# marl/l3embedding

Hardware: AMD Instinct MI355X
Metric: AVC training pairs/sec (1s audio + 224x224 frame) (higher is better)
Workload: dtype f32; 1 GPU; full cnn_L3_melspec2 AVC training step (audio+vision+fusion, fwd+bwd+Adam), batch 64 per GPU, global batch 64, fp32, inputs resident in HBM; global_batch=64, parallelism=dp1, fp32_conv=f4x4

## Files before the change

### include/l3hip.h

```cpp
#ifndef L3HIP_H
#define L3HIP_H

#include <stdint.h>

#ifdef __cplusplus
extern "C" {
#endif

#define L3_OK 0
#define L3_EINVAL (-1)
#define L3_EHIP (-2)
#define L3_ENOMEM (-3)
#define L3_ESTATE (-4)
#define L3_ECOMM (-5)

#define L3_MODEL_CNN_L3_ORIG 0
#define L3_MODEL_TINY_L3 1
#define L3_MODEL_CNN_L3_KAPREDBINPUTBN 2
#define L3_MODEL_CNN_L3_MELSPEC1 3
#define L3_MODEL_CNN_L3_MELSPEC2 4

typedef struct l3_engine l3_engine;

#define L3_DTYPE_F32 0
// ... 84 lines not shown
#define L3_COMM_ID_BYTES 128
int l3_comm_unique_id(void *id128);
int l3_comm_init(l3_engine *e, const void *id128, int world, int rank);
int l3_comm_destroy(l3_engine *e);
int l3_comm_info(const l3_engine *e, int *world, int *rank, char *library_path, int path_cap);
int l3_comm_version(void);
int l3_comm_allreduce_host(l3_engine *e, double *vals, int n, int op);
int l3_step_dp(l3_engine *e, float lr);
int l3_comm_timing(l3_engine *e, int on);
int l3_comm_timing_read(l3_engine *e, double *exposed_ms, double *span_ms, double *bucket_ms, int cap, int *steps);

int l3_grad_arena_dev(l3_engine *e, void **dev_ptr, int64_t *numel);
int l3_bucket_range(const l3_engine *e, int bucket, int64_t *offset, int64_t *numel);
int l3_bn_stats_pack_dev(l3_engine *e, void **send_dev, int64_t *numel);
int l3_bn_stats_replicas_dev(l3_engine *e, int world, void **gathered_dev);

int l3_embed_audio(l3_engine *e, const float *audio, int64_t n, int pool_h, int pool_w, float *out);
int l3_embed_vision(l3_engine *e, const float *video, int64_t n, int pool_h, int pool_w, float *out);
int64_t l3_embed_dim(const l3_engine *e, int vision, int pool_h, int pool_w);
int l3_embed_audio_frames(l3_engine *e, const float *samples, int64_t n_samples, const int64_t *table,
                          int64_t n_frames, int pool_h, int pool_w, float *out);
int l3_embed_audio_clips_resampled(l3_engine *e, const float *native, int64_t n_native, const int64_t *clips,
                                   int64_t n_clips, const double *half_window, int64_t n_window, int num_table,
                                   int64_t n_samples, const int64_t *table, int64_t n_frames, int pool_h, int pool_w,
                                   float *out);
int l3_embed_vision_frames(l3_engine *e, const uint8_t *pixels, int64_t n_bytes, const int64_t *table, int64_t n_frames,
                           int pool_h, int pool_w, float *out);

int l3_get_activation(l3_engine *e, const char *name, float *dst, int64_t numel);
int l3_activation_numel(l3_engine *e, const char *name, int64_t *numel);
int l3_sync(l3_engine *e);
int l3_profile_enable(l3_engine *e, int on);
int l3_set_tower_overlap(l3_engine *e, int on);
int l3_profile_read(l3_engine *e, int family, double *ms, int64_t *launches, double *flops);
int l3_profile_read_executed(l3_engine *e, int family, double *flops);
int l3_profile_read_bytes(l3_engine *e, int family, double *bytes);

#define L3_OP_BF16_STORED 2
#define L3_OP_BF16_STORED_OUT 3
int l3_op_conv2d_fwd_dt(int device, int dtype, const float *x, const float *w, const float *b, float *y,
                        int n, int h, int wd, int cin, int cout, int kh, int kw, int same);
int l3_op_conv2d_bwd_dt(int device, int dtype, const float *x, const float *w, const float *dy, float *dx,
                        float *dw, float *db, int n, int h, int wd, int cin, int cout, int kh, int kw, int same);
int l3_op_conv2d_fwd(int device, const float *x, const float *w, const float *b, float *y,
                     int n, int h, int wd, int cin, int cout, int kh, int kw, int same);
int l3_op_conv2d_bwd(int device, const float *x, const float *w, const float *dy,
                     float *dx, float *dw, float *db,
                     int n, int h, int wd, int cin, int cout, int kh, int kw, int same);
int l3_op_bn_relu_fwd(int device, const float *x, const float *gamma, const float *beta,
                      float *y, float *mean, float *var, int64_t rows, int c, int relu, int x_bf16);
int l3_op_bn_relu_bwd(int device, const float *x, const float *y, const float *dy,
                      const float *gamma, const float *beta, const float *mean, const float *var,
                      float *dx, float *dgamma, float *dbeta, int64_t rows, int c, int relu, int x_bf16);
int l3_op_bn_relu_pool2_fwd(int device, const float *x, const float *gamma, const float *beta, float *p,
                            float *mean, float *var, int n, int h, int wd, int c, int same, int relu_mode, int x_bf16);
int l3_op_bn_relu_pool2_bwd(int device, const float *x, const float *gamma, const float *beta, const float *dp,
                            float *dx, float *dgamma, float *dbeta, float *dbias, int n, int h, int wd, int c,
                            int same, int relu_mode, int x_bf16);
int l3_op_maxpool_fwd(int device, const float *x, float *y, int n, int h, int wd, int c,
                      int ph, int pw, int sh, int sw, int same);
int l3_op_maxpool_bwd(int device, const float *x, const float *dy, float *dx, int n, int h,
                      int wd, int c, int ph, int pw, int sh, int sw, int same);
int l3_op_frontend(int device, int model_type, const float *audio, int n, int db_max_scope, float *out);
int l3_op_gather_frames(int device, const float *samples, int64_t n_samples, const int64_t *table,
                        int64_t n_frames, float *frames);
int l3_op_image_frames(int device, const uint8_t *pixels, int64_t n_bytes, const int64_t *table, int64_t n_frames,
                       uint8_t *out_u8, float *out_f32);
int l3_op_resample(int device, const float *x, int64_t n_in, int64_t sr_orig, int64_t sr_new, const double *half_window,
                   int64_t n_window, int num_table, int64_t t0, int64_t n_out, float *y);
int l3_op_resample_clips(int device, const float *x, int64_t n_in, const int64_t *clips, int64_t n_clips, int64_t sr_new,
                         const double *half_window, int64_t n_window, int num_table, int64_t n_samples, int copy_equal,
                         float *y);
int l3_op_bn_stats_from_partials(int device, const float *part, int nblk, int c, const float *pivot, int64_t rows,
                                 float eps, float *mean, float *var);
int l3_op_conv2d_fwd_stats(int device, int dtype, const float *x, const float *w, const float *b, float *y, float *part, int *nblk,
                           float *mean, float *var, int n, int h, int wd, int cin, int cout, int kh, int kw, int same,
                           int stat_mode);
int l3_op_conv2d_dgrad_bn_bwd(int device, int dtype, const float *dy, const float *w, const float *bn_x, const float *gamma,
                              const float *beta, const float *mean, const float *var, float *dx, float *part, int *nblk,
                              float *dgamma, float *dbeta, int n, int h, int wd, int cin, int cout, int kh, int kw, int same,
                              int relu, int64_t bn_rows);
int l3_op_bn_relu_pool2_fwd_xwin(int device, const float *x, const float *gamma, const float *beta, float *p, float *mean,
                                 float *var, float *xwin, int n, int h, int wd, int c, int same, int relu_mode, int x_bf16);
int l3_op_preprocess(int device, const uint8_t *video_u8, int64_t nv, float *video,
                     const int16_t *audio_i16, int64_t na, float *audio);
int l3_op_augment_video(int device, const uint8_t *u8, int n, int h, int w, const l3_augment_params *params,
                        uint8_t *out_u8, float *out_f32);
int l3_op_augment_audio(int device, const int16_t *i16, int n, int t, const double *u, int16_t *out_i16, float *out_f32,
                        double *gains);

typedef struct l3_mlp l3_mlp;
int l3_mlp_create(int device, int D, int C, int batch, float weight_decay, uint64_t seed, l3_mlp **m);
void l3_mlp_destroy(l3_mlp *m);
int64_t l3_mlp_param_count(const l3_mlp *m);
int l3_mlp_set_data(l3_mlp *m, const float *X_train, const int32_t *y_train, int64_t n_train,
                    const float *X_valid, const int32_t *y_valid, int64_t n_valid);
int l3_mlp_epoch(l3_mlp *m, const int32_t *perm, float lr, int64_t t0, double *stats_out);
int l3_mlp_predict(l3_mlp *m, const float *X, int64_t n, float *probs_out);
int l3_mlp_get_weights(l3_mlp *m, float *dst, int64_t n);
int l3_mlp_set_weights(l3_mlp *m, const float *src, int64_t n);

int l3_op_mlp_dense_fwd(int device, const float *x, int64_t n_x, const int32_t *idx, int rows, int K, int N, const float *w,
                        const float *b, int relu, float *y);
int l3_op_mlp_dense_bwd_x(int device, const float *dy, const float *w, const float *h, int rows, int K, int N, float *dx);
int l3_op_mlp_wgrad(int device, const float *x, int64_t n_x, const int32_t *idx, int rows, int K, int N, const float *dy, float *dw,
                    float *db);
int l3_op_mlp_wgrad_adam(int device, const float *x, int64_t n_x, const int32_t *idx, int rows, int K, int N, const float *dy,
                         float *w, float *b, float *mw, float *vw, float *mb, float *vb, float weight_decay, float lr_t,
                         float *w2_out);
int l3_op_mlp_softmax_ce(int device, const float *z, const int32_t *labels, int rows, int C, float gscale, float *probs, float *dz,
                         float *ce, float *correct);
int l3_op_adam(int device, float *p, const float *g, float *m, float *v, int64_t n, int64_t n_l2, float l2x2, float lr_t);
int l3_op_adam_scaled(int device, float *p, const float *g, float *m, float *v, int64_t n, int64_t n_l2, float l2x2, float lr_t,
                      float b1, float b2, float eps, float gscale);
int l3_op_arena_fold(int device, float *acc, float *g, int64_t total, int64_t off, int64_t n, int mode);

int l3_op_head_dense_fwd(int device, const float *x, const float *w, const float *b, float *y, int B, int K, int N, int relu);
int l3_op_head_dense_bwd(int device, const float *x, const float *w, const float *dy, float *dw, float *db, float *dx, int B,
                         int K, int N);
int l3_op_softmax_ce2(int device, const float *logits, const float *labels, int B, float gscale, float *probs, float *dlogits,
                      float *stats);
int l3_op_sumsq(int device, const float *base, int64_t n_base, const int64_t *off, const int64_t *n, int count, int multi,
                float *out);
int l3_op_bn_moving_update(int device, int entries, const int32_t *c, const int64_t *slot_off, int64_t n_slots, float *moving,
                           float *biased, const float *batch, const float *gathered, int64_t n_gathered, int replicas,
                           int64_t stride, float momentum, int zero_debias, int64_t step, float *packed, int64_t n_packed);

#define L3_SVM_LINEAR 0
#define L3_SVM_POLY 1
#define L3_SVM_RBF 2
#define L3_SVM_SIGMOID 3
#define L3_SVM_DEFAULT_WS 64
#define L3_SVM_LOCAL_REL 0.1
typedef struct l3_svm_kernel {
    int32_t kind, degree;
    double gamma, coef0;
} l3_svm_kernel;
typedef struct l3_svm l3_svm;
int l3_svm_create(int device, l3_svm **m);
void l3_svm_destroy(l3_svm *m);
int l3_svm_set_data(l3_svm *m, const float *X, int64_t n, int D);
int l3_svm_fit(l3_svm *m, const l3_svm_kernel *k, double C, double tol, int64_t max_iter, int n_prob, const int64_t *prob_off,
               const int32_t *rows, const int8_t *signs, int q, double *alpha_out, double *rho_out, int64_t *updates_out,
               int32_t *outer_out, double *gap_out);
int l3_svm_fit_costs(l3_svm *m, const l3_svm_kernel *k, const double *C, double tol, int64_t max_iter, int n_prob,
                     const int64_t *prob_off, const int32_t *rows, const int8_t *signs, int q, double *alpha_out, double *rho_out,
                     int64_t *updates_out, int32_t *outer_out, double *gap_out);
int l3_svm_cv_decision(l3_svm *m, const l3_svm_kernel *k, int n_jobs, const int64_t *held_off, const int32_t *held_rows,
                       const int64_t *sv_off, const int64_t *sv_neg, const int32_t *sv_rows, const double *coef, const double *rho,
                       double *dec_out);
int l3_svm_decision(l3_svm *m, const l3_svm_kernel *k, const float *X, const int32_t *x_idx, int64_t n, int D, const float *SV,
                    const int32_t *sv_idx, int64_t n_sv, int n_class, const int64_t *sv_start, const double *coef,
                    const double *rho, double *dec_out);
int l3_op_svm_kernel_rows(int device, const l3_svm_kernel *k, const float *x, int64_t n_x, int D, const int32_t *a_idx, int na,
                          const int32_t *b_idx, int nb, float *out);
int l3_op_svm_smo(int device, const float *K, const int8_t *y, int q, double C, double eps, double local_rel, int64_t max_updates,
                  double *alpha, const double *grad, int64_t *updates_out);
int l3_svm_set_data_dev(l3_svm *m, const struct l3_feat *f, int64_t lo, int64_t hi);
int l3_svm_get_rows(l3_svm *m, const int32_t *idx, int64_t n, float *out);
int l3_svm_set_model(l3_svm *m, const l3_svm_kernel *k, const float *SV, const int32_t *sv_idx, int64_t n_sv, int D, int n_class,
                     const int64_t *sv_start, const double *coef, const double *rho, const double *probA, const double *probB);
int l3_svm_score(l3_svm *m, const float *X, const int32_t *x_idx, const struct l3_feat *feat, int64_t lo, int64_t hi, int64_t n,
                 int D, const int32_t *labels, const int64_t *files, int64_t n_files, int32_t *pred_out, double *ovr_out,
                 double *hinge_sum_out, double *proba_out, double *file_proba_out, int32_t *file_pred_out);
int l3_op_svm_tail(int device, const double *dec, int64_t n, int n_class, const double *probA, const double *probB,
                   const int32_t *labels, const int64_t *files, int64_t n_files, int32_t *pred_out, double *ovr_out,
// ... 127 lines not shown
```

### l3embedding_amd/_lib.py

```python
import ctypes as C
import os

import numpy as np

from . import _build

MODEL_IDS = {
    'cnn_L3_orig': 0,
    'tiny_L3': 1,
    'cnn_L3_kapredbinputbn': 2,
    'cnn_L3_melspec1': 3,
    'cnn_L3_melspec2': 4,
}

FAMILIES = ('conv_fwd', 'conv_dgrad', 'conv_wgrad', 'elementwise', 'frontend', 'head', 'adam')


DTYPES = {'f32': 0, 'fp32': 0, 'float32': 0, 'bf16': 1}
FP32_CONV = {'f4x4': 0, 'f2x2': 1, 'f2x2_bf16x6': 2}
DP_MOVING = {'replicas': 0, 'rank_local': 1}
OP_DTYPES = dict(DTYPES, bf16_stored=2, bf16_stored_out=3)


class L3Config(C.Structure):
# ... 46 lines not shown
                               C.POINTER(C.c_float), C.POINTER(C.c_float)]),
    'l3_upload_batch': (C.c_int, [C.c_void_p, C.c_void_p, C.c_void_p, C.c_void_p]),
    'l3_upload_batch_raw': (C.c_int, [C.c_void_p, C.c_void_p, C.c_void_p, C.c_void_p]),
    'l3_tower_step': (C.c_int, [C.c_void_p, C.c_int, C.c_int]),
    'l3_stage_batch_raw': (C.c_int, [C.c_void_p, C.c_void_p, C.c_void_p, C.c_void_p]),
    'l3_upload_batch_raw_aug': (C.c_int, [C.c_void_p, C.c_void_p, C.c_void_p, C.c_void_p, C.c_void_p, C.c_void_p]),
    'l3_stage_batch_raw_aug': (C.c_int, [C.c_void_p, C.c_void_p, C.c_void_p, C.c_void_p, C.c_void_p, C.c_void_p]),
    'l3_batch_gains': (C.c_int, [C.c_void_p, C.c_void_p]),
    'l3_step_forward': (C.c_int, [C.c_void_p, C.c_int]),
    'l3_step_bucket_count': (C.c_int, [C.c_void_p]),
    'l3_step_backward_bucket': (C.c_int, [C.c_void_p, C.c_int]),
    'l3_step_update': (C.c_int, [C.c_void_p, C.c_float, C.c_float]),
    'l3_step_resident': (C.c_int, [C.c_void_p, C.c_float]),
    'l3_replicas_upload': (C.c_int, [C.c_void_p, C.c_void_p, C.c_void_p, C.c_void_p, C.c_int]),
    'l3_replicas_upload_raw': (C.c_int, [C.c_void_p, C.c_void_p, C.c_void_p, C.c_void_p, C.c_int]),
    'l3_replicas_stage_raw': (C.c_int, [C.c_void_p, C.c_void_p, C.c_void_p, C.c_void_p, C.c_int]),
    'l3_replicas_upload_raw_aug': (C.c_int, [C.c_void_p] * 6 + [C.c_int]),
    'l3_replicas_stage_raw_aug': (C.c_int, [C.c_void_p] * 6 + [C.c_int]),
    'l3_step_replicas': (C.c_int, [C.c_void_p, C.c_float]),
    'l3_eval_replicas': (C.c_int, [C.c_void_p, C.POINTER(C.c_float), C.POINTER(C.c_float)]),
    'l3_step_results': (C.c_int, [C.c_void_p, C.POINTER(C.c_float), C.POINTER(C.c_float), C.c_void_p, C.c_void_p]),
    'l3_step_results_enqueue': (C.c_int, [C.c_void_p, C.c_int, C.c_int]),
    'l3_step_results_wait': (C.c_int, [C.c_void_p, C.c_int, C.POINTER(C.c_float), C.POINTER(C.c_float)]),
    'l3_comm_unique_id': (C.c_int, [C.c_void_p]),
    'l3_comm_init': (C.c_int, [C.c_void_p, C.c_void_p, C.c_int, C.c_int]),
    'l3_comm_destroy': (C.c_int, [C.c_void_p]),
    'l3_comm_info': (C.c_int, [C.c_void_p, C.POINTER(C.c_int), C.POINTER(C.c_int), C.c_char_p, C.c_int]),
    'l3_comm_allreduce_host': (C.c_int, [C.c_void_p, C.POINTER(C.c_double), C.c_int, C.c_int]),
    'l3_step_dp': (C.c_int, [C.c_void_p, C.c_float]),
    'l3_comm_timing': (C.c_int, [C.c_void_p, C.c_int]),
    'l3_comm_timing_read': (C.c_int, [C.c_void_p, C.POINTER(C.c_double), C.POINTER(C.c_double), C.POINTER(C.c_double), C.c_int, C.POINTER(C.c_int)]),
    'l3_grad_arena_dev': (C.c_int, [C.c_void_p, C.POINTER(C.c_void_p), C.POINTER(C.c_int64)]),
    'l3_bucket_range': (C.c_int, [C.c_void_p, C.c_int, C.POINTER(C.c_int64), C.POINTER(C.c_int64)]),
    'l3_embed_audio': (C.c_int, [C.c_void_p, C.c_void_p, C.c_int64, C.c_int, C.c_int, C.c_void_p]),
    'l3_embed_vision': (C.c_int, [C.c_void_p, C.c_void_p, C.c_int64, C.c_int, C.c_int, C.c_void_p]),
    'l3_embed_dim': (C.c_int64, [C.c_void_p, C.c_int, C.c_int, C.c_int]),
    'l3_embed_audio_frames': (C.c_int, [C.c_void_p, C.c_void_p, C.c_int64, C.c_void_p, C.c_int64, C.c_int, C.c_int,
                                        C.c_void_p]),
    'l3_embed_audio_clips_resampled': (C.c_int, [C.c_void_p, C.c_void_p, C.c_int64, C.c_void_p, C.c_int64, C.c_void_p,
                                                 C.c_int64, C.c_int, C.c_int64, C.c_void_p, C.c_int64, C.c_int, C.c_int,
                                                 C.c_void_p]),
    'l3_embed_audio_frames_dev': (C.c_int, [C.c_void_p, C.c_void_p, C.c_int64, C.c_void_p, C.c_int64, C.c_int, C.c_int,
                                            C.c_void_p, C.c_int64]),
    'l3_embed_audio_clips_resampled_dev': (C.c_int, [C.c_void_p, C.c_void_p, C.c_int64, C.c_void_p, C.c_int64, C.c_void_p,
                                                     C.c_int64, C.c_int, C.c_int64, C.c_void_p, C.c_int64, C.c_int, C.c_int,
                                                     C.c_void_p, C.c_int64]),
    'l3_embed_vision_frames': (C.c_int, [C.c_void_p, C.c_void_p, C.c_int64, C.c_void_p, C.c_int64, C.c_int, C.c_int,
                                         C.c_void_p]),
    'l3_embed_vision_frames_dev': (C.c_int, [C.c_void_p, C.c_void_p, C.c_int64, C.c_void_p, C.c_int64, C.c_int, C.c_int,
                                             C.c_void_p, C.c_int64]),
    'l3_get_activation': (C.c_int, [C.c_void_p, C.c_char_p, C.c_void_p, C.c_int64]),
    'l3_activation_numel': (C.c_int, [C.c_void_p, C.c_char_p, C.POINTER(C.c_int64)]),
    'l3_sync': (C.c_int, [C.c_void_p]),
    'l3_profile_enable': (C.c_int, [C.c_void_p, C.c_int]),
    'l3_set_tower_overlap': (C.c_int, [C.c_void_p, C.c_int]),
    'l3_profile_read_executed': (C.c_int, [C.c_void_p, C.c_int, C.POINTER(C.c_double)]),
    'l3_profile_read_bytes': (C.c_int, [C.c_void_p, C.c_int, C.POINTER(C.c_double)]),
    'l3_profile_read': (C.c_int, [C.c_void_p, C.c_int, C.POINTER(C.c_double), C.POINTER(C.c_int64),
                                  C.POINTER(C.c_double)]),
    'l3_op_conv2d_fwd': (C.c_int, [C.c_int, C.c_void_p, C.c_void_p, C.c_void_p, C.c_void_p] + [C.c_int] * 8),
    'l3_op_conv2d_fwd_dt': (C.c_int, [C.c_int, C.c_int, C.c_void_p, C.c_void_p, C.c_void_p, C.c_void_p] + [C.c_int] * 8),
    'l3_op_conv2d_bwd_dt': (C.c_int, [C.c_int, C.c_int] + [C.c_void_p] * 6 + [C.c_int] * 8),
    'l3_op_conv2d_bwd': (C.c_int, [C.c_int] + [C.c_void_p] * 6 + [C.c_int] * 8),
    'l3_op_bn_relu_fwd': (C.c_int, [C.c_int] + [C.c_void_p] * 6 + [C.c_int64, C.c_int, C.c_int, C.c_int]),
    'l3_op_bn_relu_bwd': (C.c_int, [C.c_int] + [C.c_void_p] * 10 + [C.c_int64, C.c_int, C.c_int, C.c_int]),
    'l3_op_bn_relu_pool2_fwd': (C.c_int, [C.c_int] + [C.c_void_p] * 6 + [C.c_int] * 7),
    'l3_op_bn_relu_pool2_bwd': (C.c_int, [C.c_int] + [C.c_void_p] * 8 + [C.c_int] * 7),
    'l3_op_maxpool_fwd': (C.c_int, [C.c_int, C.c_void_p, C.c_void_p] + [C.c_int] * 9),
    'l3_op_maxpool_bwd': (C.c_int, [C.c_int, C.c_void_p, C.c_void_p, C.c_void_p] + [C.c_int] * 9),
    'l3_op_frontend': (C.c_int, [C.c_int, C.c_int, C.c_void_p, C.c_int, C.c_int, C.c_void_p]),
    'l3_op_gather_frames': (C.c_int, [C.c_int, C.c_void_p, C.c_int64, C.c_void_p, C.c_int64, C.c_void_p]),
    'l3_op_image_frames': (C.c_int, [C.c_int, C.c_void_p, C.c_int64, C.c_void_p, C.c_int64, C.c_void_p, C.c_void_p]),
    'l3_op_resample': (C.c_int, [C.c_int, C.c_void_p, C.c_int64, C.c_int64, C.c_int64, C.c_void_p, C.c_int64, C.c_int,
                                 C.c_int64, C.c_int64, C.c_void_p]),
    'l3_op_resample_clips': (C.c_int, [C.c_int, C.c_void_p, C.c_int64, C.c_void_p, C.c_int64, C.c_int64, C.c_void_p, C.c_int64,
                                       C.c_int, C.c_int64, C.c_int, C.c_void_p]),
    'l3_op_bn_stats_from_partials': (C.c_int, [C.c_int, C.c_void_p, C.c_int, C.c_int, C.c_void_p, C.c_int64, C.c_float,
                                               C.c_void_p, C.c_void_p]),
    'l3_op_conv2d_fwd_stats': (C.c_int, [C.c_int, C.c_int] + [C.c_void_p] * 5 + [C.POINTER(C.c_int), C.c_void_p, C.c_void_p] +
                               [C.c_int] * 9),
    'l3_op_conv2d_dgrad_bn_bwd': (C.c_int, [C.c_int, C.c_int] + [C.c_void_p] * 9 + [C.POINTER(C.c_int), C.c_void_p, C.c_void_p] +
                                  [C.c_int] * 9 + [C.c_int64]),
    'l3_op_bn_relu_pool2_fwd_xwin': (C.c_int, [C.c_int] + [C.c_void_p] * 7 + [C.c_int] * 7),
    'l3_op_preprocess': (C.c_int, [C.c_int, C.c_void_p, C.c_int64, C.c_void_p, C.c_void_p, C.c_int64, C.c_void_p]),
    'l3_op_augment_video': (C.c_int, [C.c_int, C.c_void_p, C.c_int, C.c_int, C.c_int, C.c_void_p, C.c_void_p, C.c_void_p]),
    'l3_op_augment_audio': (C.c_int, [C.c_int, C.c_void_p, C.c_int, C.c_int, C.c_void_p, C.c_void_p, C.c_void_p, C.c_void_p]),
    'l3_mlp_create': (C.c_int, [C.c_int, C.c_int, C.c_int, C.c_int, C.c_float, C.c_uint64, C.POINTER(C.c_void_p)]),
    'l3_mlp_destroy': (None, [C.c_void_p]),
    'l3_mlp_param_count': (C.c_int64, [C.c_void_p]),
    'l3_mlp_set_data': (C.c_int, [C.c_void_p, C.c_void_p, C.c_void_p, C.c_int64, C.c_void_p, C.c_void_p, C.c_int64]),
    'l3_mlp_epoch': (C.c_int, [C.c_void_p, C.c_void_p, C.c_float, C.c_int64, C.POINTER(C.c_double)]),
    'l3_mlp_predict': (C.c_int, [C.c_void_p, C.c_void_p, C.c_int64, C.c_void_p]),
    'l3_mlp_get_weights': (C.c_int, [C.c_void_p, C.c_void_p, C.c_int64]),
    'l3_mlp_set_weights': (C.c_int, [C.c_void_p, C.c_void_p, C.c_int64]),
    'l3_op_mlp_dense_fwd': (C.c_int, [C.c_int, C.c_void_p, C.c_int64, C.c_void_p, C.c_int, C.c_int, C.c_int, C.c_void_p,
                                      C.c_void_p, C.c_int, C.c_void_p]),
    'l3_op_mlp_dense_bwd_x': (C.c_int, [C.c_int, C.c_void_p, C.c_void_p, C.c_void_p, C.c_int, C.c_int, C.c_int, C.c_void_p]),
    'l3_op_mlp_wgrad': (C.c_int, [C.c_int, C.c_void_p, C.c_int64, C.c_void_p, C.c_int, C.c_int, C.c_int, C.c_void_p,
                                  C.c_void_p, C.c_void_p]),
    'l3_op_mlp_wgrad_adam': (C.c_int, [C.c_int, C.c_void_p, C.c_int64, C.c_void_p, C.c_int, C.c_int, C.c_int, C.c_void_p]
                             + [C.c_void_p] * 6 + [C.c_float, C.c_float, C.c_void_p]),
    'l3_op_mlp_softmax_ce': (C.c_int, [C.c_int, C.c_void_p, C.c_void_p, C.c_int, C.c_int, C.c_float] + [C.c_void_p] * 4),
    'l3_op_adam': (C.c_int, [C.c_int] + [C.c_void_p] * 4 + [C.c_int64, C.c_int64, C.c_float, C.c_float]),
    'l3_op_adam_scaled': (C.c_int, [C.c_int] + [C.c_void_p] * 4 + [C.c_int64, C.c_int64] + [C.c_float] * 6),
    'l3_op_arena_fold': (C.c_int, [C.c_int, C.c_void_p, C.c_void_p, C.c_int64, C.c_int64, C.c_int64, C.c_int]),
    'l3_op_head_dense_fwd': (C.c_int, [C.c_int] + [C.c_void_p] * 4 + [C.c_int] * 4),
    'l3_op_head_dense_bwd': (C.c_int, [C.c_int] + [C.c_void_p] * 6 + [C.c_int] * 3),
    'l3_op_softmax_ce2': (C.c_int, [C.c_int, C.c_void_p, C.c_void_p, C.c_int, C.c_float] + [C.c_void_p] * 3),
    'l3_op_sumsq': (C.c_int, [C.c_int, C.c_void_p, C.c_int64, C.c_void_p, C.c_void_p, C.c_int, C.c_int, C.c_void_p]),
    'l3_op_bn_moving_update': (C.c_int, [C.c_int, C.c_int, C.c_void_p, C.c_void_p, C.c_int64] + [C.c_void_p] * 4
                               + [C.c_int64, C.c_int, C.c_int64, C.c_float, C.c_int, C.c_int64, C.c_void_p, C.c_int64]),
    'l3_svm_create': (C.c_int, [C.c_int, C.POINTER(C.c_void_p)]),
    'l3_svm_destroy': (None, [C.c_void_p]),
    'l3_svm_set_data': (C.c_int, [C.c_void_p, C.c_void_p, C.c_int64, C.c_int]),
    'l3_svm_fit': (C.c_int, [C.c_void_p, C.c_void_p, C.c_double, C.c_double, C.c_int64, C.c_int] + [C.c_void_p] * 3
                   + [C.c_int] + [C.c_void_p] * 5),
    'l3_svm_fit_costs': (C.c_int, [C.c_void_p, C.c_void_p, C.c_void_p, C.c_double, C.c_int64, C.c_int] + [C.c_void_p] * 3
                         + [C.c_int] + [C.c_void_p] * 5),
    'l3_svm_cv_decision': (C.c_int, [C.c_void_p, C.c_void_p, C.c_int] + [C.c_void_p] * 8),
    'l3_op_svm_sigmoid_train': (C.c_int, [C.c_int, C.c_int] + [C.c_void_p] * 6),
    'l3_svm_decision': (C.c_int, [C.c_void_p, C.c_void_p, C.c_void_p, C.c_void_p, C.c_int64, C.c_int, C.c_void_p, C.c_void_p,
                                  C.c_int64, C.c_int] + [C.c_void_p] * 4),
    'l3_op_svm_kernel_rows': (C.c_int, [C.c_int, C.c_void_p, C.c_void_p, C.c_int64, C.c_int, C.c_void_p, C.c_int, C.c_void_p,
                                        C.c_int, C.c_void_p]),
    'l3_op_svm_smo': (C.c_int, [C.c_int, C.c_void_p, C.c_void_p, C.c_int, C.c_double, C.c_double, C.c_double, C.c_int64,
                                C.c_void_p, C.c_void_p, C.c_void_p]),
    'l3_svm_set_data_dev': (C.c_int, [C.c_void_p, C.c_void_p, C.c_int64, C.c_int64]),
    'l3_svm_get_rows': (C.c_int, [C.c_void_p, C.c_void_p, C.c_int64, C.c_void_p]),
    'l3_svm_set_model': (C.c_int, [C.c_void_p, C.c_void_p, C.c_void_p, C.c_void_p, C.c_int64, C.c_int, C.c_int] + [C.c_void_p] * 5),
    'l3_svm_score': (C.c_int, [C.c_void_p, C.c_void_p, C.c_void_p, C.c_void_p, C.c_int64, C.c_int64, C.c_int64, C.c_int, C.c_void_p,
                               C.c_void_p, C.c_int64] + [C.c_void_p] * 6),
    'l3_op_svm_tail': (C.c_int, [C.c_int, C.c_void_p, C.c_int64, C.c_int, C.c_void_p, C.c_void_p, C.c_void_p, C.c_void_p, C.c_int64]
                       + [C.c_void_p] * 8),
    'l3_vggish_create': (C.c_int, [C.c_int, C.c_int, C.POINTER(C.c_void_p)]),
    'l3_vggish_destroy': (None, [C.c_void_p]),
    'l3_vggish_batch': (C.c_int, [C.c_void_p]),
    'l3_vggish_set_conv': (C.c_int, [C.c_void_p, C.c_int]),
    'l3_vggish_set_weight': (C.c_int, [C.c_void_p, C.c_char_p, C.c_void_p, C.c_int64]),
    'l3_vggish_set_pca': (C.c_int, [C.c_void_p, C.c_void_p, C.c_void_p]),
    'l3_vggish_embed_clips_resampled': (C.c_int, [C.c_void_p, C.c_void_p, C.c_int64, C.c_void_p, C.c_int64, C.c_void_p, C.c_int64,
                                                  C.c_int, C.c_int64, C.c_void_p, C.c_int64, C.c_void_p, C.c_int64, C.c_int,
                                                  C.c_void_p]),
    'l3_op_vggish_logmel': (C.c_int, [C.c_int, C.c_void_p, C.c_int64, C.c_void_p, C.c_int64, C.c_void_p]),
    'l3_op_vggish_conv1': (C.c_int, [C.c_int, C.c_void_p, C.c_int64, C.c_void_p, C.c_int64, C.c_void_p, C.c_void_p, C.c_void_p]),
    'l3_op_vggish_bias_relu': (C.c_int, [C.c_int, C.c_void_p, C.c_void_p, C.c_void_p] + [C.c_int] * 5),
    'l3_op_vggish_postprocess': (C.c_int, [C.c_int, C.c_void_p, C.c_int64, C.c_void_p, C.c_void_p, C.c_int, C.c_void_p]),
    'l3_op_vggish_conv': (C.c_int, [C.c_int, C.c_int, C.c_void_p, C.c_void_p, C.c_void_p, C.c_void_p] + [C.c_int] * 6),
    'l3_feat_create': (C.c_int, [C.c_int, C.c_void_p, C.c_int64, C.c_int64, C.POINTER(C.c_void_p)]),
    'l3_feat_alloc': (C.c_int, [C.c_int, C.c_int64, C.c_int64, C.POINTER(C.c_void_p)]),
    'l3_feat_destroy': (None, [C.c_void_p]),
    'l3_feat_shape': (C.c_int, [C.c_void_p, C.POINTER(C.c_int64), C.POINTER(C.c_int64)]),
    'l3_feat_download': (C.c_int, [C.c_void_p, C.c_int64, C.c_int64, C.c_void_p]),
    'l3_feat_assemble': (C.c_int, [C.c_int, C.c_void_p, C.c_int64, C.POINTER(C.c_void_p)]),
    'l3_feat_gather': (C.c_int, [C.c_void_p, C.c_void_p, C.c_int64]),
    'l3_feat_split': (C.c_int, [C.c_void_p, C.c_void_p, C.c_int64, C.c_void_p, C.c_int64, C.POINTER(C.c_void_p), C.POINTER(C.c_void_p)]),
    'l3_feat_minmax': (C.c_int, [C.c_void_p, C.c_void_p, C.c_void_p]),
    'l3_feat_affine32': (C.c_int, [C.c_void_p, C.c_void_p, C.c_void_p]),
    'l3_feat_moments': (C.c_int, [C.c_void_p, C.c_void_p, C.c_void_p]),
    'l3_feat_standardize': (C.c_int, [C.c_void_p, C.c_void_p, C.c_void_p]),
    'l3_feat_file_stats': (C.c_int, [C.c_void_p, C.c_void_p, C.c_int64]),
    'l3_mlp_set_data_dev': (C.c_int, [C.c_void_p, C.c_void_p, C.c_int64, C.c_int64, C.c_void_p, C.c_void_p, C.c_int64, C.c_int64,
                                      C.c_void_p]),
    'l3_mlp_predict_dev': (C.c_int, [C.c_void_p, C.c_void_p, C.c_int64, C.c_int64, C.c_void_p]),
    'l3_mlp_predict_files_dev': (C.c_int, [C.c_void_p, C.c_void_p, C.c_void_p, C.c_int64, C.c_void_p, C.c_void_p]),
    'l3_op_file_mean': (C.c_int, [C.c_int, C.c_void_p, C.c_int64, C.c_int, C.c_void_p, C.c_int64, C.c_void_p, C.c_void_p]),
    'l3_mlp_group_create': (C.c_int, [C.c_int, C.c_int, C.c_int, C.c_int, C.c_int, C.c_void_p, C.c_void_p, C.POINTER(C.c_void_p)]),
# ... 517 lines not shown
    check(lib.l3_op_conv2d_fwd_stats(device, OP_DTYPES[dtype], None, None, None, None, None, C.byref(nblk), None, None, *dims))
    y = np.empty((n, ho, wo, cout), np.float32)
    part = np.empty((nblk.value, 2, cout), np.float32)
    mean, var = np.empty(cout, np.float32), np.empty(cout, np.float32)
    check(lib.l3_op_conv2d_fwd_stats(device, OP_DTYPES[dtype], _ptr(x), _ptr(w), _ptr(b), _ptr(y), _ptr(part), C.byref(nblk),
                                     _ptr(mean), _ptr(var), *dims))
    assert nblk.value == part.shape[0]
    return y, part, mean, var


def op_conv2d_dgrad_bn_bwd(dy, w, same, bn_x, gamma, beta, mean, var, relu, bn_rows=None, dtype='f32', device=0):
    lib = load()
    dy, w, bn_x = _f32(dy), _f32(w), _f32(bn_x)
    n, h, wd, cin = bn_x.shape
    kh, kw, wci, cout = w.shape
    ho, wo = (h, wd) if same else (h - kh + 1, wd - kw + 1)
    assert wci == cin and dy.shape == (n, ho, wo, cout)
    rows = int(bn_rows) if bn_rows is not None else n * h * wd
    dims = (n, h, wd, cin, cout, kh, kw, int(same), int(relu), rows)
    nblk = C.c_int(0)
    check(lib.l3_op_conv2d_dgrad_bn_bwd(device, OP_DTYPES[dtype], *([None] * 9), C.byref(nblk), None, None, *dims))
    dx = np.empty_like(bn_x)
    part = np.empty((nblk.value, 2, cin), np.float32)
    dg, db = np.empty(cin, np.float32), np.empty(cin, np.float32)
    vecs = [_f32(v) for v in (gamma, beta, mean, var)]
    assert all(v.shape == (cin,) for v in vecs)
    check(lib.l3_op_conv2d_dgrad_bn_bwd(device, OP_DTYPES[dtype], _ptr(dy), _ptr(w), _ptr(bn_x), *[_ptr(v) for v in vecs], _ptr(dx),
                                        _ptr(part), C.byref(nblk), _ptr(dg), _ptr(db), *dims))
    return dx, part, dg, db


def op_bn_relu_fwd(x, gamma, beta, relu, device=0, x_bf16=False, out_bf16=False):
    lib = load()
    x = _f32(x)
    c = x.shape[-1]
    rows = x.size // c
    y = np.empty_like(x)
    mean, var = np.empty((c,), np.float32), np.empty((c,), np.float32)
    check(lib.l3_op_bn_relu_fwd(device, _ptr(x), _ptr(_f32(gamma)), _ptr(_f32(beta)), _ptr(y), _ptr(mean),
                                _ptr(var), rows, c, int(relu), int(x_bf16) | (4 if out_bf16 else 0)))
    return y, mean, var


def op_bn_relu_bwd(x, y, dy, gamma, mean, var, relu, device=0, beta=None, x_bf16=False, out_bf16=False):
    lib = load()
    x, y, dy = _f32(x), _f32(y), _f32(dy)
    c = x.shape[-1]
    rows = x.size // c
    dx = np.empty_like(x)
    dg, db = np.empty((c,), np.float32), np.empty((c,), np.float32)
    check(lib.l3_op_bn_relu_bwd(device, _ptr(x), _ptr(y), _ptr(dy), _ptr(_f32(gamma)), _ptr(_f32(beta)), _ptr(_f32(mean)),
                                _ptr(_f32(var)), _ptr(dx), _ptr(dg), _ptr(db), rows, c, int(relu), int(x_bf16) | (4 if out_bf16 else 0)))
    return dx, dg, db


def op_bn_relu_pool2_fwd(x, gamma, beta, same, device=0, relu_mode=1, x_bf16=False, want_xwin=False, out_bf16=False):
    lib = load()
    flags = int(x_bf16) | (4 if out_bf16 else 0)
    x = _f32(x)
    n, h, wd, c = x.shape
    p = np.empty((n, _pool_out(h, 2, 2, same), _pool_out(wd, 2, 2, same), c), np.float32)
    mean, var = np.empty((c,), np.float32), np.empty((c,), np.float32)
    if want_xwin:
        xwin = np.empty_like(p)
        check(lib.l3_op_bn_relu_pool2_fwd_xwin(device, _ptr(x), _ptr(_f32(gamma)), _ptr(_f32(beta)), _ptr(p), _ptr(mean), _ptr(var),
                                               _ptr(xwin), n, h, wd, c, int(same), int(relu_mode), flags))
        return p, mean, var, xwin
    check(lib.l3_op_bn_relu_pool2_fwd(device, _ptr(x), _ptr(_f32(gamma)), _ptr(_f32(beta)), _ptr(p), _ptr(mean),
                                      _ptr(var), n, h, wd, c, int(same), int(relu_mode), flags))
    return p, mean, var


def op_bn_relu_pool2_bwd(x, gamma, beta, dp, same, device=0, relu_mode=1, x_bf16=False, out_bf16=False):
    lib = load()
    x, dp = _f32(x), _f32(dp)
    n, h, wd, c = x.shape
    dx = np.empty_like(x)
    dg, db, dbias = (np.empty((c,), np.float32) for _ in range(3))
    check(lib.l3_op_bn_relu_pool2_bwd(device, _ptr(x), _ptr(_f32(gamma)), _ptr(_f32(beta)), _ptr(dp), _ptr(dx),
                                      _ptr(dg), _ptr(db), _ptr(dbias), n, h, wd, c, int(same), int(relu_mode), int(x_bf16) | (4 if out_bf16 else 0)))
    return dx, dg, db, dbias


def _pool_out(h, p, s, same):
    return -(-h // s) if same else (h - p) // s + 1


def op_maxpool_fwd(x, ph, pw, sh, sw, same, device=0):
    lib = load()
    x = _f32(x)
    n, h, wd, c = x.shape
    y = np.empty((n, _pool_out(h, ph, sh, same), _pool_out(wd, pw, sw, same), c), np.float32)
    check(lib.l3_op_maxpool_fwd(device, _ptr(x), _ptr(y), n, h, wd, c, ph, pw, sh, sw, int(same)))
    return y


def op_maxpool_bwd(x, dy, ph, pw, sh, sw, same, device=0):
    lib = load()
    x, dy = _f32(x), _f32(dy)
    n, h, wd, c = x.shape
    dx = np.empty_like(x)
    check(lib.l3_op_maxpool_bwd(device, _ptr(x), _ptr(dy), _ptr(dx), n, h, wd, c, ph, pw, sh, sw, int(same)))
    return dx


def op_bn_stats_from_partials(part, pivot, rows, eps=1e-3, device=0):
    lib = load()
    part, pivot = _f32(part), _f32(pivot)
    nblk, two, c = part.shape
    assert two == 2 and pivot.shape == (c,)
    mean, var = np.empty(c, np.float32), np.empty(c, np.float32)
    check(lib.l3_op_bn_stats_from_partials(device, _ptr(part), nblk, c, _ptr(pivot), int(rows), float(eps), _ptr(mean), _ptr(var)))
    return mean, var


def op_frontend(model_type, audio, db_max_scope='sample', device=0):
    lib = load()
    a = _f32(audio)
    n = a.shape[0]
    probe = {'cnn_L3_orig': (257, 197), 'tiny_L3': (257, 198), 'cnn_L3_kapredbinputbn': (257, 197),
             'cnn_L3_melspec1': (128, 199), 'cnn_L3_melspec2': (256, 199)}[model_type]
    out = np.empty((n, probe[0], probe[1], 1), np.float32)
    check(lib.l3_op_frontend(device, MODEL_IDS[model_type], _ptr(a), n, 0 if db_max_scope == 'sample' else 1, _ptr(out)))
    return out


def op_gather_frames(samples, table, device=0):
    lib = load()
    s = np.ascontiguousarray(samples, dtype=np.float32).reshape(-1)
    t = np.ascontiguousarray(table, dtype=np.int64).reshape(-1, 3)
    if s.size == 0:
        s = np.zeros(1, np.float32)[:0]
    out = np.empty((t.shape[0], 48000), np.float32)
    check(lib.l3_op_gather_frames(device, _ptr(s), s.size, _ptr(t), t.shape[0], _ptr(out)))
    return out


def op_image_frames(pixels, table, device=0, want_u8=True, want_f32=True):
    lib = load()
    p = np.ascontiguousarray(pixels, dtype=np.uint8).reshape(-1)
    t = np.ascontiguousarray(table, dtype=np.int64).reshape(-1, 7)
    if p.size == 0:
        p = np.zeros(1, np.uint8)[:0]
    u8 = np.empty((t.shape[0], 224, 224, 3), np.uint8) if want_u8 else None
    f32 = np.empty((t.shape[0], 224, 224, 3), np.float32) if want_f32 else None
    check(lib.l3_op_image_frames(device, _ptr(p), p.size, _ptr(t), t.shape[0], _ptr(u8), _ptr(f32)))
    return u8, f32


def op_resample(x, sr_orig, sr_new, half_window, num_table, t0=0, n_out=None, device=0):
    lib = load()
    a = np.ascontiguousarray(x, dtype=np.float32).reshape(-1)
    w = np.ascontiguousarray(half_window, dtype=np.float64).reshape(-1)
    if n_out is None:
        n_out = max(0, int(a.size * (float(sr_new) / sr_orig)) - int(t0)) if sr_orig > 0 else 0
    out = np.empty(max(int(n_out), 0), np.float32)
    check(lib.l3_op_resample(device, _ptr(a), a.size, int(sr_orig), int(sr_new), _ptr(w), w.size, int(num_table), int(t0),
                             int(n_out), _ptr(out)))
    return out


def op_resample_clips(x, clips, sr_new, half_window, num_table, n_samples, copy_equal=False, device=0):
    lib = load()
    a = np.ascontiguousarray(x, dtype=np.float32).reshape(-1)
    c = np.ascontiguousarray(clips, dtype=np.int64).reshape(-1, 6)
    w = np.ascontiguousarray(half_window, dtype=np.float64).reshape(-1)
# ... 1014 lines not shown
```

### l3embedding_amd/csrc/bn_fused.hip

```cpp
#include "kernels.h"
#include "device_common.h"

namespace l3 {



__device__ __forceinline__ void store_quad(void* base, int64_t q, f32x4 v, int obf) {
    if (obf) {
        bf16x4 h;
        h[0] = (__bf16)v.x; h[1] = (__bf16)v.y; h[2] = (__bf16)v.z; h[3] = (__bf16)v.w;
        __builtin_nontemporal_store(h, reinterpret_cast<bf16x4*>(base) + q);
    } else {
        __builtin_nontemporal_store(v, reinterpret_cast<f32x4*>(base) + q);
    }
}

template <bool XBF>
__device__ __forceinline__ f32x4 load_quad(const void* base, int64_t q) {
    if constexpr (XBF) {
        const u32x2 r = __builtin_nontemporal_load(reinterpret_cast<const u32x2*>(base) + q);
        return f32x4{__uint_as_float(r.x << 16), __uint_as_float(r.x & 0xffff0000u), __uint_as_float(r.y << 16),
                     __uint_as_float(r.y & 0xffff0000u)};
    } else {
        return __builtin_nontemporal_load(reinterpret_cast<const f32x4*>(base) + q);
// ... 495 lines not shown
                    return o;
                };
                const f32x4 o00 = gate2(A * d00 + (B * x00 + Cc), r00);
                store_quad(dx, base, o00, obf);
                a0 += o00;
                if (w1ok) {
                    const f32x4 o = gate2(A * d01 + (B * x01 + Cc), r01);
                    store_quad(dx, base + dw, o, obf);
                    a0 += o;
                }
                if (h1ok) {
                    const f32x4 o = gate2(A * d10 + (B * x10 + Cc), r10);
                    store_quad(dx, base + dh, o, obf);
                    a0 += o;
                }
                if (h1ok && w1ok) {
                    const f32x4 o = gate2(A * d11 + (B * x11 + Cc), r11);
                    store_quad(dx, base + dh + dw, o, obf);
                    a0 += o;
                }
            }
        }
    }
    if (part != nullptr) block_write_partials(a0, a0, part, g.C4);
}

struct SumFinal {
    float* out;
    __device__ void operator()(int c, double s0, double) const { out[c] = (float)s0; }
};

void bn_bwd_fast(const float* x, const float* scale, const float* shift, const float* mean, const float* var,
                 const float* gamma, const float* dy, int pooled, int N, int H, int W, int C, int Ho, int Wo,
                 int64_t dy_batch_stride, float* dx, float* dgamma, float* dbeta, float* dbias, float* scratch,
                 float eps, int relu, int training, hipStream_t s, int dx_bf16, int x_bf16, int dy_bf16,
                 const float* ready_part, int ready_blocks) {
    const int64_t rows = (int64_t)N * H * W;
    const int64_t n4 = rows * (C / 4);
    Pool2Geom g = make_pool2(N, H, W, C, pooled ? Ho : H, pooled ? Wo : W, pooled ? dy_batch_stride : (int64_t)H * W * C);
    float* part = scratch;
    float* cA = scratch + (size_t)FAST_MAX_BLOCKS * 2 * C;
    float* cB = cA + C;
    float* cC = cB + C;
    const void* xv = (const void*)x;
    const void* dyv = (const void*)dy;
    const f32x4* sc4 = reinterpret_cast<const f32x4*>(scale);
    const f32x4* sh4 = reinterpret_cast<const f32x4*>(shift);
    const int64_t work_r = pooled ? (int64_t)N * Ho * Wo * (C / 4) : n4;
    const int nb_r = fast_blocks(work_r);
    const int variant = (pooled ? 4 : 0) | (x_bf16 ? 2 : 0) | (dy_bf16 ? 1 : 0);
    using ReduceFn = void (*)(const void*, const void*, const f32x4*, const f32x4*, const f32x4*, const f32x4*, float*, int64_t,
                              Pool2Geom, float, int);
    static const ReduceFn reduce_fns[8] = {
        bn_bwd_reduce_fast_kernel<false, false, false>, bn_bwd_reduce_fast_kernel<false, false, true>,
        bn_bwd_reduce_fast_kernel<false, true, false>,  bn_bwd_reduce_fast_kernel<false, true, true>,
        bn_bwd_reduce_fast_kernel<true, false, false>,  bn_bwd_reduce_fast_kernel<true, false, true>,
        bn_bwd_reduce_fast_kernel<true, true, false>,   bn_bwd_reduce_fast_kernel<true, true, true>};
    if (ready_part != nullptr) {
        launch_fast_final(BwdFinal{gamma, mean, var, dgamma, dbeta, cA, cB, cC, 1.0 / (double)rows, eps, training}, ready_part,
                          ready_blocks, C, s);
    } else {
        hipLaunchKernelGGL(reduce_fns[variant], dim3(nb_r), dim3(FB), 0, s, xv, dyv, sc4, sh4, reinterpret_cast<const f32x4*>(mean),
                           reinterpret_cast<const f32x4*>(var), part, n4, g, eps, relu);
        launch_fast_final(BwdFinal{gamma, mean, var, dgamma, dbeta, cA, cB, cC, 1.0 / (double)rows, eps, training}, part,
                          nb_r, C, s);
    }
    if (dx == nullptr) return;
    const int64_t work_a = pooled ? (int64_t)N * g.Hc * g.Wc * (C / 4) : n4;
    const int nb_a = fast_blocks(work_a);
    float* part2 = dbias ? part : nullptr;
    using ApplyFn = void (*)(const void*, const void*, const f32x4*, const f32x4*, const f32x4*, const f32x4*, const f32x4*, void*,
                             float*, int64_t, Pool2Geom, int, int);
    static const ApplyFn apply_fns[8] = {
        bn_bwd_apply_fast_kernel<false, false, false>, bn_bwd_apply_fast_kernel<false, false, true>,
        bn_bwd_apply_fast_kernel<false, true, false>,  bn_bwd_apply_fast_kernel<false, true, true>,
        bn_bwd_apply_fast_kernel<true, false, false>,  bn_bwd_apply_fast_kernel<true, false, true>,
        bn_bwd_apply_fast_kernel<true, true, false>,   bn_bwd_apply_fast_kernel<true, true, true>};
    hipLaunchKernelGGL(apply_fns[variant], dim3(nb_a), dim3(FB), 0, s, xv, dyv, sc4, sh4, reinterpret_cast<const f32x4*>(cA),
                       reinterpret_cast<const f32x4*>(cB), reinterpret_cast<const f32x4*>(cC), (void*)dx, part2, n4, g, relu,
                       dx_bf16);
    if (dbias) launch_fast_final(SumFinal{dbias}, part, nb_a, C, s);
}

}
```

### l3embedding_amd/csrc/elementwise.hip

```cpp
#include <algorithm>

#include "kernels.h"

namespace l3 {

static constexpr int RED_BLOCK = 256;
static constexpr int RED_MAX_BLOCKS = 1024;
static constexpr int SMALLC_MAX = 16;

static inline int red_blocks(int64_t rows, int C) {
    int rows_per_pass = (C % 4 == 0 && C >= 4 && C <= 1024) ? (RED_BLOCK / (C / 4) > 0 ? RED_BLOCK / (C / 4) : 1) : RED_BLOCK;
    int64_t b = (rows + (int64_t)rows_per_pass * 16 - 1) / ((int64_t)rows_per_pass * 16);
    if (b < 1) b = 1;
    if (b > RED_MAX_BLOCKS) b = RED_MAX_BLOCKS;
    return (int)b;
}

size_t colreduce_scratch_floats(int64_t rows, int C) {
    const size_t a = (size_t)red_blocks(rows, C) * 2 * (size_t)(C < 4 ? 4 : C) + 64;
    const size_t b = bn_fast_ok(C) ? bn_fast_scratch_floats(C) : 0;
    return a > b ? a : b;
}

template <class F>
// ... 442 lines not shown
            }
        }
        y[(size_t)n * g.out_batch_stride + ((size_t)ho * g.Wo + wo) * g.C + c] = best;
    }
}
typedef float gp4 __attribute__((ext_vector_type(4)));
__device__ __forceinline__ void gp_scan(const float* __restrict__ xb, int P, int C, int pg, float best[4], int arg[4]) {
#pragma unroll
    for (int e = 0; e < 4; ++e) {
        best[e] = -INFINITY;
        arg[e] = 0x7fffffff;
    }
    for (int p = pg; p < P; p += 16) {
        const gp4 v = *reinterpret_cast<const gp4*>(xb + (size_t)p * C);
#pragma unroll
        for (int e = 0; e < 4; ++e)
            if (v[e] > best[e] || arg[e] == 0x7fffffff) {
                best[e] = v[e];
                arg[e] = p;
            }
    }
}
__device__ __forceinline__ void gp_merge(float (*sb)[64], int (*sa)[64], int pg, int cq, float best[4], int arg[4]) {
#pragma unroll
    for (int e = 0; e < 4; ++e) {
        sb[pg][cq * 4 + e] = best[e];
        sa[pg][cq * 4 + e] = arg[e];
    }
    __syncthreads();
    if (pg == 0) {
#pragma unroll
        for (int e = 0; e < 4; ++e) {
            float b = best[e];
            int a = arg[e];
            for (int k = 1; k < 16; ++k) {
                const float vb = sb[k][cq * 4 + e];
                const int va = sa[k][cq * 4 + e];
                if (vb > b || (vb == b && va < a)) {
                    b = vb;
                    a = va;
                }
            }
            sb[0][cq * 4 + e] = b;
            sa[0][cq * 4 + e] = a;
        }
    }
    __syncthreads();
}
__global__ __launch_bounds__(256) void global_maxpool_fwd_kernel(const float* __restrict__ x, float* __restrict__ y, int P,
                                                                 int C, int64_t out_batch_stride) {
    __shared__ float sb[16][64];
    __shared__ int sa[16][64];
    const int cb = blockIdx.x % (C / 64), n = blockIdx.x / (C / 64);
    const int cq = threadIdx.x & 15, pg = threadIdx.x >> 4;
    float best[4];
    int arg[4];
    gp_scan(x + (size_t)n * P * C + cb * 64 + cq * 4, P, C, pg, best, arg);
    gp_merge(sb, sa, pg, cq, best, arg);
    if (threadIdx.x < 64) y[(size_t)n * out_batch_stride + cb * 64 + threadIdx.x] = sb[0][threadIdx.x];
}
__global__ __launch_bounds__(256) void global_maxpool_bwd_kernel(const float* __restrict__ x, const float* __restrict__ dy,
                                                                 float* __restrict__ dx, int P, int C,
                                                                 int64_t out_batch_stride) {
    __shared__ float sb[16][64];
    __shared__ int sa[16][64];
    const int cb = blockIdx.x % (C / 64), n = blockIdx.x / (C / 64);
    const int cq = threadIdx.x & 15, pg = threadIdx.x >> 4;
    float best[4];
    int arg[4];
    const size_t base = (size_t)n * P * C + cb * 64 + cq * 4;
    gp_scan(x + base, P, C, pg, best, arg);
    gp_merge(sb, sa, pg, cq, best, arg);
    const gp4 d = *reinterpret_cast<const gp4*>(dy + (size_t)n * out_batch_stride + cb * 64 + cq * 4);
    int am[4];
#pragma unroll
    for (int e = 0; e < 4; ++e) am[e] = sa[0][cq * 4 + e];
    for (int p = pg; p < P; p += 16) {
        gp4 o;
#pragma unroll
        for (int e = 0; e < 4; ++e) o[e] = p == am[e] ? d[e] : 0.f;
        *reinterpret_cast<gp4*>(dx + base + (size_t)p * C) = o;
    }
}
static bool is_global_pool(const PoolGeom& g) {
    return g.Ho == 1 && g.Wo == 1 && g.padT == 0 && g.padL == 0 && g.ph == g.H && g.pw == g.W && g.C % 64 == 0 &&
           g.out_batch_stride % 4 == 0;
}

void maxpool_fwd(const float* x, float* y, const PoolGeom& g, hipStream_t s) {
    if (is_global_pool(g)) {
        hipLaunchKernelGGL(global_maxpool_fwd_kernel, dim3(g.N * (g.C / 64)), dim3(256), 0, s, x, y, g.H * g.W, g.C,
                           (int64_t)g.out_batch_stride);
        return;
    }
    const int64_t total = (int64_t)g.N * g.Ho * g.Wo * g.C;
    hipLaunchKernelGGL(maxpool_fwd_kernel, dim3(ew_blocks(total)), dim3(256), 0, s, x, y, g);
}
__global__ __launch_bounds__(256) void maxpool_bwd_kernel(const float* x, const float* dy, float* dx, PoolGeom g) {
    const int64_t total = (int64_t)g.N * g.Ho * g.Wo * g.C;
    for (int64_t i = (int64_t)blockIdx.x * 256 + threadIdx.x; i < total; i += (int64_t)gridDim.x * 256) {
        const int c = (int)(i % g.C);
        int64_t r = i / g.C;
        const int wo = (int)(r % g.Wo);
        r /= g.Wo;
        const int ho = (int)(r % g.Ho);
        const int n = (int)(r / g.Ho);
        const int h0 = ho * g.sh - g.padT, w0 = wo * g.sw - g.padL;
        float best = -INFINITY;
        int ba = -1, bb = -1;
        for (int a = 0; a < g.ph; ++a) {
            const int h = h0 + a;
            if ((unsigned)h >= (unsigned)g.H) continue;
            for (int b = 0; b < g.pw; ++b) {
                const int w = w0 + b;
                if ((unsigned)w >= (unsigned)g.W) continue;
                const float v = x[((size_t)(n * g.H + h) * g.W + w) * g.C + c];
                if (ba < 0 || v > best) { best = v; ba = a; bb = b; }
            }
        }
        const float d = dy[(size_t)n * g.out_batch_stride + ((size_t)ho * g.Wo + wo) * g.C + c];
        for (int a = 0; a < g.ph; ++a) {
            const int h = h0 + a;
            if ((unsigned)h >= (unsigned)g.H) continue;
            for (int b = 0; b < g.pw; ++b) {
                const int w = w0 + b;
                if ((unsigned)w >= (unsigned)g.W) continue;
                dx[((size_t)(n * g.H + h) * g.W + w) * g.C + c] = (a == ba && b == bb) ? d : 0.f;
            }
        }
    }
}
void maxpool_bwd(const float* x, const float* dy, float* dx, const PoolGeom& g, hipStream_t s) {
    if (is_global_pool(g)) {
        hipLaunchKernelGGL(global_maxpool_bwd_kernel, dim3(g.N * (g.C / 64)), dim3(256), 0, s, x, dy, dx, g.H * g.W,
                           g.C, (int64_t)g.out_batch_stride);
        return;
    }
    const bool covers = (g.Ho - 1) * g.sh - g.padT + g.ph >= g.H && (g.Wo - 1) * g.sw - g.padL + g.pw >= g.W &&
                        g.sh == g.ph && g.sw == g.pw;
    if (!covers) (void)hipMemsetAsync(dx, 0, (size_t)g.N * g.H * g.W * g.C * sizeof(float), s);
    const int64_t total = (int64_t)g.N * g.Ho * g.Wo * g.C;
    hipLaunchKernelGGL(maxpool_bwd_kernel, dim3(ew_blocks(total)), dim3(256), 0, s, x, dy, dx, g);
}

__global__ __launch_bounds__(256) void bn_xhat_ones_kernel(const float* __restrict__ x, const float* __restrict__ mean,
                                                           const float* __restrict__ var, float eps, float* __restrict__ xa,
                                                           int64_t rows, int C) {
    const int C1 = C + 1;
    const int64_t total = rows * C1;
    for (int64_t i = (int64_t)blockIdx.x * 256 + threadIdx.x; i < total; i += (int64_t)gridDim.x * 256) {
        const int c = (int)(i % C1);
        const int64_t r = i / C1;
        xa[i] = c == C ? 1.f : (x[r * C + c] - mean[c]) * (1.f / sqrtf(var[c] + eps));
    }
}
void bn_xhat_ones(const float* x, const float* mean, const float* var, float eps, float* xa, int64_t rows, int C,
                  hipStream_t s) {
    hipLaunchKernelGGL(bn_xhat_ones_kernel, dim3(ew_blocks(rows * (C + 1))), dim3(256), 0, s, x, mean, var, eps, xa, rows, C);
}

__global__ __launch_bounds__(256) void first_conv_grads_kernel(const float* __restrict__ gaug, const float* __restrict__ w,
                                                               const float* __restrict__ gamma, const float* __restrict__ beta,
                                                               float* __restrict__ dw, float* __restrict__ dgamma,
                                                               float* __restrict__ dbeta, float* __restrict__ dbias, int taps,
                                                               int C, int Co) {
    __shared__ double red[2][256];
    const int t = threadIdx.x;
// ... 327 lines not shown
```

### l3embedding_amd/csrc/engine.hip

```cpp
#include <hip/hip_runtime.h>
#include "knobs.h"

#include <cmath>
#include <cstdio>
#include <cstdlib>
#include <cstring>
#include <map>
#include <string>
#include <vector>

#include "../../include/l3hip.h"
#include "comm.h"
#include "conv_path.h"
#include "featprep.h"
#include "kernels.h"

namespace {

using namespace l3;

static thread_local std::string g_create_error;

constexpr float BN_EPS = 1e-3f;
constexpr float BN_MOMENTUM = 0.99f;
constexpr float L2_WEIGHT = 1e-5f;
constexpr float ADAM_B1 = 0.9f, ADAM_B2 = 0.999f, ADAM_EPS = 1e-8f;
constexpr int AUDIO_T = 48000;

enum ParamKind { PK_KERNEL, PK_BIAS, PK_GAMMA, PK_BETA, PK_MMEAN, PK_MVAR, PK_CONST };
enum OpKind { OP_CONV, OP_BN, OP_RELU, OP_POOL, OP_FLATTEN };
enum Family { F_CONV_FWD, F_CONV_DGRAD, F_CONV_WGRAD, F_ELEMWISE, F_FRONTEND, F_HEAD, F_ADAM, F_COUNT };

struct Tensor {
    float* d = nullptr;
    float* g = nullptr;
    int N = 0, H = 0, W = 0, C = 0;
    int64_t batch_stride = 0;
    bool alias = false;
    bool d_bf16 = false, g_bf16 = false;
    int64_t numel() const { return (int64_t)N * H * W * C; }
    int64_t rows() const { return (int64_t)N * H * W; }
};

struct Param {
    std::string name;
    int ndim = 0;
    int64_t shape[4] = {1, 1, 1, 1};
    bool trainable = false;
    int kind = 0;
    int64_t numel = 0;
    int bucket = 0;
    float* d = nullptr;
    float* g = nullptr;
};

enum FirstWgrad { FW_NONE, FW_AUG, FW_AUG_DEFERRED };
struct ConvPlan {
    ConvStorage st;
    ConvFwdPath fwd;
    int stat_mode = 0;
    FirstWgrad aug = FW_NONE;
    ConvWgradPath wgrad;
    bool colsum = false;
    ConvDgradPath dgrad;
    int bwd_bn = -1;
    double fwd_bytes = 0.0, wg_bytes = 0.0, dg_bytes = 0.0;
};
enum BnStats { BS_PARTIALS, BS_FAST, BS_PLAIN, BS_MOVING };
enum BnBwd { BB_BY_FIRST_CONV, BB_FAST_POOLED, BB_FAST, BB_FAST_DEFERRED, BB_PLAIN };
struct BnPlan {
    BnStats stats = BS_MOVING;
    int stat_blocks = 0;
    BnBwd bwd = BB_PLAIN;
    int bwd_blocks = 0;
    double fwd_bytes = 0.0, bwd_bytes = 0.0;
};

struct Op {
    OpKind kind;
    std::string name;
    int in = 0, out = 0;
    int block = 0, bucket = 0;
    int kh = 0, kw = 0, cout = 0;
    bool same = false;
    ConvGeom geom{};
    ConvGeom dgeom{};
    int p_kernel = -1, p_bias = -1;
    float* wflip = nullptr;
    float *wino_uf = nullptr, *wino_ud = nullptr;
    int in_bn = -1;
    bool fused_first = false;
    bool defer_apply = false;
    int bn_defer = -1;
    float *xaug = nullptr, *gaug = nullptr;
    ConvGeom ageom{};
    int bn_follow = -1;
    bool need_dx = true;
    int dy_to_bn = -1;
    float* xwin = nullptr;
    int p_gamma = -1, p_beta = -1, p_mmean = -1, p_mvar = -1;
    bool fused_relu = false;
    bool prerelu = false;
    int fuse_pool = -1;
    int bias_param = -1;
    bool fused_into_bn = false;
    bool bias_by_bn = false;
    float *mean = nullptr, *var = nullptr, *scale = nullptr, *shift = nullptr;
    float *biased_mean = nullptr, *biased_var = nullptr;
    PoolGeom pg{};
    ConvPlan cp{};
    BnPlan bp{};
};

struct Tower {
    std::string prefix;
    std::vector<Tensor> t;
    std::vector<Op> ops;
    int nblocks = 0;
    int emb_conv_op = -1;
    bool training = false;
};

struct FrontendDef {
    int n_dft, n_hop, same, n_mels, sqrt_out, db, loglambda;
    const char* layer_name;
};

struct ProfRec {
    int family;
    hipEvent_t a, b;
    double flops;
    double executed;
    double bytes;
    const char* tag;
};

}

struct l3_engine {
    l3_config cfg{};
    int B = 0;
    hipStream_t stream = nullptr;
    bool own_stream = false;
    hipStream_t side = nullptr;
    hipEvent_t ev_fork = nullptr, ev_join = nullptr;
    float *red_scratch2 = nullptr, *wg_scratch2 = nullptr;
    float *stat_scratch = nullptr, *stat_scratch2 = nullptr;
    size_t stat_max = 0;
    float* w4_tail = nullptr;
    bool overlap = true;
    BnMovingEntry* bn_table = nullptr;
    int bn_table_n = 0, bn_table_max_c = 0;
    std::string err;
    l3::DeviceBufs bufs;

    std::vector<Param> params;
    std::map<std::string, int> pindex;
    float *arena_p = nullptr, *arena_g = nullptr, *arena_m = nullptr, *arena_v = nullptr;
    int64_t n_train = 0;
    struct Segment { int64_t off, n; bool l2; };
    std::vector<Segment> segments;
    struct Bucket { int64_t off, n; };
    std::vector<Bucket> buckets;
    int64_t adam_t = 0;
    int64_t bn_step = 0;

    Tower vis, aud;
    FrontendDef fe{};
    FrontendCfg fcfg{};
    int p_real = -1, p_imag = -1, p_mel = -1;
    bool consts_dirty = true;
    float *wdft = nullptr, *melw = nullptr, *frames = nullptr, *spec = nullptr, *smax = nullptr;
    bool dft_consts_done = false;
    float *dft_win = nullptr, *dft_b1 = nullptr, *dft_b2 = nullptr, *dft_tw = nullptr, *dft_y = nullptr, *dft_a2 = nullptr, *dft_nyq = nullptr;
    int *mel_start = nullptr, *mel_len = nullptr, *mel_off = nullptr;
    int64_t melw_cap = 0;

    float *video = nullptr, *audio = nullptr, *labels = nullptr;
    l3::BatchFeed feed;
    float* res_host = nullptr;
    float* res_sum = nullptr;
    bool res_reduced[2] = {false, false};
    bool res_pending[2] = {false, false};
    hipEvent_t ev_res[2] = {nullptr, nullptr};
    hipEvent_t ev_res_a = nullptr, ev_res_b = nullptr;
    hipEvent_t ev_step[2] = {nullptr, nullptr};
// ... 359 lines not shown
    }
    assign_blocks(e->vis);
    assign_blocks(e->aud);
    const Tensor& vo = e->vis.t.back();
    const Tensor& ao = e->aud.t.back();
    e->nv = vo.H * vo.W * vo.C;
    e->na = ao.H * ao.W * ao.C;
    e->head = (mt == L3_MODEL_TINY_L3) ? 64 : 128;
    add_param(e, "dense_1/kernel", {e->nv + e->na, e->head}, true, PK_KERNEL, &e->p_w1);
    add_param(e, "dense_1/bias", {e->head}, true, PK_BIAS, &e->p_b1);
    add_param(e, "dense_2/kernel", {e->head, 2}, true, PK_KERNEL, &e->p_w2);
    add_param(e, "dense_2/bias", {2}, true, PK_BIAS, &e->p_b2);

    for (Tower* tw : {&e->vis, &e->aud}) {
        bool any = false;
        for (auto& op : tw->ops) {
            if (op.kind == OP_CONV) op.need_dx = any;
            if (op.kind == OP_CONV || op.kind == OP_BN) any = true;
        }
    }
    const int bnbwd_fuse = knob_int("L3_BNBWD_FUSE", 1);
    if (bnbwd_fuse)
        for (Tower* tw : {&e->vis, &e->aud})
            for (size_t i = 0; i < tw->ops.size(); ++i) {
                Op& cv = tw->ops[i];
                if (cv.kind != OP_CONV || !cv.need_dx) continue;
                for (size_t j = 0; j < i; ++j) {
                    const Op& bn = tw->ops[j];
                    if (bn.kind == OP_BN && bn.out == cv.in && bn.fuse_pool < 0 && !bn.prerelu && bn.block == cv.block &&
                        bn_fast_ok(tw->t[bn.in].C))
                        cv.dy_to_bn = (int)j;
                }
            }
    static const int first_fused = knob_int("L3_FIRST_FUSED", 1);
    if (first_fused)
        for (Tower* tw : {&e->vis, &e->aud})
            for (size_t i = 1; i < tw->ops.size(); ++i) {
                Op& op = tw->ops[i];
                if (op.kind != OP_CONV) continue;
                Op& bn = tw->ops[i - 1];
                if (bn.kind == OP_BN && bn.in == 0 && !bn.fused_relu && bn.block == op.block && op.same &&
                    tw->t[op.in].C <= 7) {
                    op.in_bn = (int)i - 1;
                    bn.fused_first = true;
                    op.ageom = op.geom;
                    op.ageom.Cin = op.geom.Cin + 1;
                }
                break;
            }
    const int nbv = e->vis.nblocks, nba = e->aud.nblocks;
    for (auto& op : e->vis.ops) op.bucket = 1 + (nbv - 1 - op.block);
    for (auto& op : e->aud.ops) op.bucket = 1 + nbv + (nba - 1 - op.block);
    for (Tower* tw : {&e->vis, &e->aud})
        for (auto& op : tw->ops) {
            for (int pi : {op.p_kernel, op.p_bias, op.p_gamma, op.p_beta})
                if (pi >= 0) e->params[pi].bucket = op.bucket;
        }
    for (int pi : {e->p_w1, e->p_b1, e->p_w2, e->p_b2}) e->params[pi].bucket = 0;
    for (Tower* tw : {&e->vis, &e->aud})
        for (size_t i = 0; i < tw->ops.size(); ++i) {
            Op& op = tw->ops[i];
            if (op.kind != OP_BN || !bn_fast_ok(tw->t[op.in].C)) continue;
            if (i > 0 && tw->ops[i - 1].kind == OP_CONV) {
                op.bias_param = tw->ops[i - 1].p_bias;
                tw->ops[i - 1].bias_by_bn = true;
                tw->ops[i - 1].bn_follow = (int)i;
            }
            const bool pool_next = i + 2 < tw->ops.size() && tw->ops[i + 1].kind == OP_POOL &&
                                   tw->ops[i + 1].pg.ph == 2 && tw->ops[i + 1].pg.pw == 2 && tw->ops[i + 1].pg.sh == 2 &&
                                   tw->ops[i + 1].pg.sw == 2 && tw->ops[i + 1].pg.padT == 0 && tw->ops[i + 1].pg.padL == 0;
            if (op.fused_relu && pool_next) {
                op.fuse_pool = (int)i + 1;
                tw->ops[i + 1].fused_into_bn = true;
            } else if (!op.fused_relu && pool_next && i >= 2 && tw->ops[i - 1].kind == OP_RELU &&
                       tw->ops[i - 2].kind == OP_CONV) {
                op.prerelu = true;
                op.in = tw->ops[i - 2].out;
                tw->ops[i - 1].fused_into_bn = true;
                op.bias_param = tw->ops[i - 2].p_bias;
                tw->ops[i - 2].bias_by_bn = true;
                tw->ops[i - 2].bn_follow = (int)i;
                op.fuse_pool = (int)i + 1;
                tw->ops[i + 1].fused_into_bn = true;
            }
        }
    const int first_wg_fuse = knob_int("L3_FIRST_WG_FUSE", 1);
    if (first_wg_fuse)
        for (Tower* tw : {&e->vis, &e->aud})
            for (auto& cv : tw->ops) {
                if (cv.kind != OP_CONV || cv.in_bn < 0 || cv.bn_follow < 0 || !cv.bias_by_bn) continue;
                Op& bn = tw->ops[cv.bn_follow];
                if (bn.kind == OP_BN && bn.fuse_pool < 0 && !bn.prerelu && bn.in == cv.out && bn_fast_ok(cv.cout) &&
                    conv_first_wgrad_ok(cv.ageom)) {
                    bn.defer_apply = true;
                    cv.bn_defer = cv.bn_follow;
                }
            }
    const int pooled_fuse = knob_int("L3_BNBWD_FUSE_POOLED", 1);
    if (bnbwd_fuse && pooled_fuse)
        for (Tower* tw : {&e->vis, &e->aud})
            for (size_t i = 0; i < tw->ops.size(); ++i) {
                Op& cv = tw->ops[i];
                if (cv.kind != OP_CONV || !cv.need_dx || cv.dy_to_bn >= 0) continue;
                for (size_t j = 0; j < i; ++j) {
                    const Op& bn = tw->ops[j];
                    if (bn.kind == OP_BN && bn.fuse_pool >= 0 && tw->ops[bn.fuse_pool].out == cv.in && (bn.fused_relu != bn.prerelu) &&
                        bn_fast_ok(tw->t[bn.in].C))
                        cv.dy_to_bn = (int)j;
                }
            }
    return L3_OK;
}

void host_dft_kernels(int n_dft, std::vector<float>& real, std::vector<float>& imag) {
    const int nb = n_dft / 2 + 1;
    real.assign((size_t)n_dft * nb, 0.f);
    imag.assign((size_t)n_dft * nb, 0.f);
    const double two_pi = 2.0 * M_PI;
    for (int t = 0; t < n_dft; ++t) {
        const float win = (float)(0.5 - 0.5 * std::cos(two_pi * (double)t / (double)n_dft));
        for (int k = 0; k < nb; ++k) {
            const double w = (double)k * two_pi / (double)n_dft;
            real[(size_t)t * nb + k] = (float)(std::cos(w * (double)t) * (double)win);
            imag[(size_t)t * nb + k] = (float)(-std::sin(w * (double)t) * (double)win);
        }
    }
}

void host_mel_basis(int sr, int n_fft, int n_mels, std::vector<float>& freq2mel ) {
    const int nb = n_fft / 2 + 1;
    auto hz2mel = [](double f) { return 2595.0 * std::log10(1.0 + f / 700.0); };
    auto mel2hz = [](double m) { return 700.0 * (std::pow(10.0, m / 2595.0) - 1.0); };
    const double fmax = (double)sr / 2.0;
    std::vector<double> mel_f(n_mels + 2);
    const double m0 = hz2mel(0.0), m1 = hz2mel(fmax);
    for (int i = 0; i < n_mels + 2; ++i) {
        const double m = (i == n_mels + 1) ? m1 : m0 + (double)i * ((m1 - m0) / (double)(n_mels + 1));
        mel_f[i] = mel2hz(m);
    }
    freq2mel.assign((size_t)nb * n_mels, 0.f);
    for (int i = 0; i < n_mels; ++i) {
        const double fd0 = mel_f[i + 1] - mel_f[i], fd1 = mel_f[i + 2] - mel_f[i + 1];
        const double enorm = 2.0 / (mel_f[i + 2] - mel_f[i]);
        for (int j = 0; j < nb; ++j) {
            const double fj = (j == nb - 1) ? fmax : (double)j * (fmax / (double)(nb - 1));
            const double lower = -(mel_f[i] - fj) / fd0;
            const double upper = (mel_f[i + 2] - fj) / fd1;
            double w = lower < upper ? lower : upper;
            if (w < 0.0) w = 0.0;
            freq2mel[(size_t)j * n_mels + i] = (float)(w * enorm);
        }
    }
}

struct Rng {
    uint64_t s;
    explicit Rng(uint64_t seed) : s(seed ? seed : 0x9E3779B97F4A7C15ull) {}
    uint64_t next() {
        uint64_t z = (s += 0x9E3779B97F4A7C15ull);
        z = (z ^ (z >> 30)) * 0xBF58476D1CE4E5B9ull;
        z = (z ^ (z >> 27)) * 0x94D049BB133111EBull;
        return z ^ (z >> 31);
    }
    double uni() { return ((double)(next() >> 11) + 0.5) * (1.0 / 9007199254740992.0); }
    double normal() {
        const double u1 = uni(), u2 = uni();
// ... 248 lines not shown
                tw->t[cv.in].d_bf16 = true;
                tw->t[cv.out].g_bf16 = true;
                if (bf16_out && (int)ci != tw->emb_conv_op) tw->t[cv.out].d_bf16 = true;
                if (bf16_dgrad_out) tw->t[cv.in].g_bf16 = true;
            }
    if (e->cfg.dtype == L3_DTYPE_BF16 && bf16_storage && bf16_out)
        for (Tower* tw : {&e->vis, &e->aud})
            for (size_t ci = 0; ci < tw->ops.size(); ++ci) {
                Op& cv = tw->ops[ci];
                if (cv.kind == OP_CONV && conv_first_ok(cv.geom) && cv.bn_follow >= 0 && cv.bias_by_bn &&
                    (int)ci != tw->emb_conv_op)
                    tw->t[cv.out].d_bf16 = true;
            }
    auto t_floats = [](const Tensor& t, bool bf16) { return bf16 ? (size_t)(t.numel() + 1) / 2 : (size_t)t.numel(); };
    size_t red_max = 1024, wg_max = 16;
    size_t& stat_max = e->stat_max;
    for (int ti = 0; ti < 2; ++ti) {
        Tower& tw = ti == 0 ? e->vis : e->aud;
        tw.t[0].d = ti == 0 ? e->video : nullptr;
        if (ti == 1) {
            if ((rc = dev_alloc_t(e, &tw.t[0].d, (size_t)tw.t[0].numel()))) return rc;
        }
        const int64_t concat_off = ti == 0 ? 0 : e->nv;
        for (size_t oi = 0; oi < tw.ops.size(); ++oi) {
            Op& op = tw.ops[oi];
            Tensor& y = tw.t[op.out];
            const bool last = oi + 1 == tw.ops.size();
            if (last) {
                y.d = e->h0 + concat_off;
                y.g = e->dh0 + concat_off;
                y.batch_stride = D;
                y.alias = true;
                if (op.kind == OP_POOL) op.pg.out_batch_stride = D;
            } else if ((op.kind == OP_BN && op.fuse_pool >= 0) || (op.kind == OP_RELU && op.fused_into_bn)) {
                if (op.kind == OP_BN) {
                    bool wanted = false;
                    for (size_t ci = 0; ci < tw.ops.size(); ++ci)
                        if (tw.ops[ci].kind == OP_CONV && tw.ops[ci].dy_to_bn == (int)oi) wanted = true;
                    const Tensor& pl = tw.t[tw.ops[op.fuse_pool].out];
                    if (wanted && (rc = dev_alloc_t(e, &op.xwin, t_floats(pl, tw.t[op.in].d_bf16)))) return rc;
                }
            } else {
                if ((rc = dev_alloc_t(e, &y.d, t_floats(y, y.d_bf16)))) return rc;
                if ((rc = dev_alloc_t(e, &y.g, t_floats(y, y.g_bf16)))) return rc;
            }
            const Tensor& x = tw.t[op.in];
            if (op.kind == OP_CONV) {
                if ((rc = dev_alloc_t(e, &op.wflip, (size_t)e->params[op.p_kernel].numel))) return rc;
                if (conv_wino_floats(op.geom) && (rc = dev_alloc_t(e, &op.wino_uf, conv_wino_floats(op.geom)))) return rc;
                {
                    const size_t sf = (size_t)conv_wino_stat_blocks_max(op.geom) * 2 * op.geom.Cout;
                    if (sf > stat_max) stat_max = sf;
                    const size_t sb = (size_t)conv_bf16_stat_blocks(op.geom) * 2 * op.geom.Cout;
                    if (e->cfg.dtype == L3_DTYPE_BF16 && sb > stat_max) stat_max = sb;
                    const size_t s1 = (size_t)conv_first_stat_blocks(op.geom) * 2 * op.geom.Cout;
                    if (s1 > stat_max) stat_max = s1;
                    const size_t sd = op.dy_to_bn >= 0 ? (size_t)conv_wino_stat_blocks_max(op.dgeom) * 2 * op.dgeom.Cout : 0;
                    if (sd > stat_max) stat_max = sd;
                    const size_t sdb = op.dy_to_bn >= 0 && e->cfg.dtype == L3_DTYPE_BF16
                                           ? (size_t)conv_bf16_stat_blocks(op.dgeom) * 2 * op.dgeom.Cout : 0;
                    if (sdb > stat_max) stat_max = sdb;
                }
                if (op.need_dx && conv_wino_floats(op.dgeom) &&
                    (rc = dev_alloc_t(e, &op.wino_ud, conv_wino_floats(op.dgeom))))
                    return rc;
                const size_t w = conv_wgrad_scratch_floats(op.geom);
                if (w > wg_max) wg_max = w;
                if (op.in_bn >= 0) {
                    if ((rc = dev_alloc_t(e, &op.xaug, (size_t)x.rows() * op.ageom.Cin))) return rc;
                    if ((rc = dev_alloc_t(e, &op.gaug, (size_t)op.kh * op.kw * op.ageom.Cin * op.cout))) return rc;
                    const size_t wa = conv_wgrad_scratch_floats(op.ageom);
                    if (wa > wg_max) wg_max = wa;
                }
                const size_t r = colreduce_scratch_floats(y.rows(), y.C);
                if (r > red_max) red_max = r;
            } else if (op.kind == OP_BN) {
                const int C = x.C;
                for (float** p : {&op.mean, &op.var, &op.scale, &op.shift, &op.biased_mean, &op.biased_var}) {
                    if ((rc = dev_alloc_t(e, p, (size_t)(C + 3) / 4 * 4))) return rc;
                    HIPCHK(e, hipMemset(*p, 0, (size_t)(C + 3) / 4 * 4 * 4));
                }
                const size_t r = colreduce_scratch_floats(x.rows(), C);
                if (r > red_max) red_max = r;
            }
        }
    }
    if (e->vis.ops.back().kind != OP_POOL || e->aud.ops.back().kind != OP_POOL) {
        e->err = "tower must end in a pooling layer";
        return L3_EINVAL;
    }
    if ((rc = dev_alloc_t(e, &e->red_scratch, red_max))) return rc;
    if ((rc = dev_alloc_t(e, &e->wg_scratch, wg_max))) return rc;
    if ((rc = dev_alloc_t(e, &e->sq_scratch, 2048))) return rc;
    if (stat_max && (rc = dev_alloc_t(e, &e->stat_scratch, stat_max))) return rc;
    {
        bool any_w4 = false;
        for (Tower* tw : {&e->vis, &e->aud})
            for (auto& op : tw->ops)
                if (op.kind == OP_CONV && (op.wino_uf || op.wino_ud)) any_w4 = true;
        if (any_w4 && e->cfg.dtype != L3_DTYPE_BF16 && (rc = dev_alloc_t(e, &e->w4_tail, conv_wino4_tail_scratch_bytes() / sizeof(float)))) return rc;
    }
    if (e->side) {
        if ((rc = dev_alloc_t(e, &e->red_scratch2, red_max))) return rc;
        if ((rc = dev_alloc_t(e, &e->wg_scratch2, wg_max))) return rc;
        if (stat_max && (rc = dev_alloc_t(e, &e->stat_scratch2, stat_max))) return rc;
    }
    return L3_OK;
}

int run_frontend(l3_engine* e) {
    int rc = rebuild_consts(e);
    if (rc) return rc;
    const FrontendCfg& f = e->fcfg;
    const int B = e->B;
    const int M = B * f.n_frames;
    if (f.factored) {
        const int N1 = f.N1, N2 = f.N2;
        const int form = knob_int("L3_DFT_FACTORED", 1);
        if (form != 2 && f.n_mels > 0 && N1 == 32 && N2 == 64) {
            const double m1 = (double)M * N2, m2 = (double)M * N1;
            ProfScope ps(e, F_FRONTEND, 2.0 * M * (double)f.n_dft * 2.0 * f.n_freq + 2.0 * M * (double)f.n_freq * f.n_mels, nullptr,
                         2.0 * m1 * N1 * 2 * N1 + 2.0 * m2 * 2 * N2 * N2);
            dft_fused(e->audio, e->dft_win, e->dft_b1, e->dft_b2, e->dft_tw, e->melw, e->mel_start, e->mel_len, e->mel_off, e->aud.t[0].d, B,
                      AUDIO_T, f, e->stream);
            if (f.db) db_normalize(e->aud.t[0].d, e->smax, B, e->aud.t[0].batch_stride, e->cfg.db_max_scope, e->stream);
            return L3_OK;
        }
        {
            ProfScope ps(e, F_FRONTEND, 0.0);
            dft_pack_frames(e->audio, e->dft_win, e->frames, B, AUDIO_T, f, e->stream);
        }
        {
            const double m1 = (double)M * N2, m2 = (double)M * N1;
            ProfScope ps(e, F_FRONTEND, 2.0 * M * (double)f.n_dft * 2.0 * f.n_freq, nullptr, 2.0 * m1 * N1 * 2 * N1 + 2.0 * m2 * 2 * N2 * N2);
            const ConvGeom g1{1, 1, M * N2, N1, 1, M * N2, 2 * N1, 1, 1, 0, 0}, g2{1, 1, M * N1, 2 * N2, 1, M * N1, N2, 1, 1, 0, 0};
            conv_fwd(e->frames, e->dft_b1, nullptr, e->dft_y, g1, e->stream);
            dft_twiddle(e->dft_y, e->dft_tw, e->dft_a2, e->dft_nyq, M, f, e->stream);
            conv_fwd(e->dft_a2, e->dft_b2, nullptr, e->spec, g2, e->stream);
        }
    } else if (f.folded) {
        float* fe = e->frames;
        float* fo = e->frames + (size_t)M * f.ke;
        {
            ProfScope ps(e, F_FRONTEND, 0.0);
            frame_audio_folded(e->audio, fe, fo, B, AUDIO_T, f, e->stream);
        }
        ProfScope ps(e, F_FRONTEND, 2.0 * M * (double)f.n_dft * 2.0 * f.n_freq, nullptr,
                     2.0 * M * (double)(f.ke + f.ko) * f.nc);
        const ConvGeom ge{1, 1, M, f.ke, 1, M, f.nc, 1, 1, 0, 0}, go{1, 1, M, f.ko, 1, M, f.nc, 1, 1, 0, 0};
        conv_fwd(fe, e->wdft, nullptr, e->spec, ge, e->stream);
        conv_fwd(fo, e->wdft + (size_t)f.ke * f.nc, nullptr, e->spec + (size_t)M * f.nc, go, e->stream);
    } else {
        {
            ProfScope ps(e, F_FRONTEND, 0.0);
            frame_audio(e->audio, e->frames, B, AUDIO_T, f, e->stream);
        }
        ConvGeom g{1, 1, M, f.n_dft, 1, M, f.ncols_pad, 1, 1, 0, 0};
        ProfScope ps(e, F_FRONTEND, 2.0 * M * (double)f.n_dft * 2.0 * f.n_freq);
        conv_fwd(e->frames, e->wdft, nullptr, e->spec, g, e->stream);
    }
    {
        ProfScope ps(e, F_FRONTEND, f.n_mels ? 2.0 * B * f.n_frames * (double)f.n_freq * f.n_mels : 0.0);
        spec_to_features(e->spec, e->melw, e->mel_start, e->mel_len, e->mel_off, e->aud.t[0].d, B, f, e->stream, e->dft_nyq);
        if (f.db) db_normalize(e->aud.t[0].d, e->smax, B, e->aud.t[0].batch_stride, e->cfg.db_max_scope, e->stream);
    }
    return L3_OK;
}

static inline double act_bytes(const Tensor& t) { return (double)t.numel() * (t.d_bf16 ? 2.0 : 4.0); }
static inline double grad_bytes(const Tensor& t) { return (double)t.numel() * (t.g_bf16 ? 2.0 : 4.0); }

int plan_tower(l3_engine* e, Tower& tw, bool training, int solo) {
    static const int epi_stats = knob_int("L3_EPILOGUE_STATS", 1);
    const bool bf16 = e->cfg.dtype == L3_DTYPE_BF16;
    tw.training = training;
    auto fits = [&](const Op& cv, int blocks, int C) {
        if ((size_t)blocks * 2 * C <= e->stat_max) return true;
        e->err = cv.name + ": " + std::to_string(blocks) + " partial blocks of " + std::to_string(C) + " channels exceed the statistics scratch (" +
                 std::to_string(e->stat_max) + " floats)";
        return false;
    };
    auto defers = [&](const Op& bn) {
        return training && bn.defer_apply && bn.fuse_pool < 0 && bn_fast_ok(tw.t[bn.in].C) && tw.t[bn.in].d_bf16 == tw.t[bn.out].g_bf16;
    };
    for (auto& op : tw.ops) op.bp = BnPlan{};
    for (auto& op : tw.ops) {
        if (op.kind != OP_CONV) continue;
        op.geom.solo = op.dgeom.solo = solo;
        op.geom.dynamic = op.dgeom.dynamic = e->comm != nullptr ? 1 : 0;
        float* ts = solo ? e->w4_tail : nullptr;
        op.geom.tail_scratch = op.dgeom.tail_scratch = ts;
        op.geom.tail_scratch_bytes = op.dgeom.tail_scratch_bytes = ts ? conv_wino4_tail_scratch_bytes() : 0;

        const Tensor &x = tw.t[op.in], &y = tw.t[op.out];
        const double wbytes = (double)e->params[op.p_kernel].numel * 4.0;
        ConvPlan& p = op.cp = ConvPlan{};
        p.st = ConvStorage{bf16, x.d_bf16, y.d_bf16, y.g_bf16, x.g_bf16};
        p.fwd = conv_resolve_fwd(op.geom, p.st, op.wino_uf != nullptr);
        p.fwd_bytes = act_bytes(x) + act_bytes(y) + wbytes;
        const int nblk = conv_fwd_stat_blocks(p.fwd, op.geom);
        if (epi_stats && training && op.bn_follow >= 0 && e->stat_max > 0 && nblk > 0) {
            if (!fits(op, nblk, op.geom.Cout)) return L3_ESTATE;
            p.stat_mode = tw.ops[op.bn_follow].prerelu ? 2 : 1;
            tw.ops[op.bn_follow].bp.stat_blocks = nblk;
        }
        if (training && op.in_bn >= 0) {
            const Op* fb = op.bn_defer >= 0 && defers(tw.ops[op.bn_defer]) ? &tw.ops[op.bn_defer] : nullptr;
            p.aug = fb ? FW_AUG_DEFERRED : FW_AUG;
            p.wg_bytes = (double)x.rows() * op.ageom.Cin * 4.0 + (fb ? act_bytes(tw.t[fb->in]) + grad_bytes(tw.t[fb->out]) : grad_bytes(y));
            continue;
        }
        p.wgrad = conv_resolve_wgrad(op.geom, p.st);
        p.wg_bytes = act_bytes(x) + grad_bytes(y) + wbytes;
        p.colsum = !op.bias_by_bn;
        if (!op.need_dx) continue;
        p.dgrad = conv_resolve_dgrad(op.geom, op.dgeom, p.st, op.wino_ud != nullptr);
        p.dg_bytes = grad_bytes(y) + grad_bytes(x) + wbytes;
        Op* bn = training && op.dy_to_bn >= 0 && e->stat_max > 0 ? &tw.ops[op.dy_to_bn] : nullptr;
        if (bn != nullptr && bn->fuse_pool >= 0 && (bn->xwin == nullptr || x.batch_stride != (int64_t)x.H * x.W * x.C)) bn = nullptr;
        if (bn == nullptr) continue;
        const int blocks = conv_dgrad_bn_blocks(p.dgrad, op.dgeom, x.g_bf16, tw.t[bn->in].d_bf16);
        if (blocks < 0) continue;
        if (!fits(op, blocks, op.dgeom.Cout)) return L3_ESTATE;
        p.bwd_bn = op.dy_to_bn;
        bn->bp.bwd_blocks = blocks;
    }
    for (auto& op : tw.ops) {
        if (op.kind != OP_BN) continue;
        const Tensor &x = tw.t[op.in], &y = tw.t[op.out];
        const Tensor& out = op.fuse_pool >= 0 ? tw.t[tw.ops[op.fuse_pool].out] : y;
        BnPlan& p = op.bp;
        p.stats = !training ? BS_MOVING : p.stat_blocks > 0 ? BS_PARTIALS : op.prerelu || x.d_bf16 ? BS_FAST : BS_PLAIN;
        p.bwd = training && op.fused_first ? BB_BY_FIRST_CONV : !bn_fast_ok(x.C) ? BB_PLAIN : op.fuse_pool >= 0 ? BB_FAST_POOLED
                : defers(op) ? BB_FAST_DEFERRED : BB_FAST;
        p.fwd_bytes = (!training ? 0.0 : p.stat_blocks > 0 ? (double)p.stat_blocks * 2 * x.C * 4 : act_bytes(x)) + act_bytes(x) + act_bytes(out);
        if (p.bwd == BB_BY_FIRST_CONV) p.fwd_bytes += act_bytes(x) + (double)x.rows() * (&op + 1)->ageom.Cin * 4.0;
        if (op.fuse_pool >= 0 && training && op.xwin != nullptr) p.fwd_bytes += (double)out.numel() * (x.d_bf16 ? 2.0 : 4.0);
        p.bwd_bytes = p.bwd == BB_PLAIN ? 2.0 * (act_bytes(x) + grad_bytes(y)) + grad_bytes(x)
                                        : (p.bwd_blocks > 0 ? (double)p.bwd_blocks * 2 * x.C * 4 : act_bytes(x) + grad_bytes(out)) +
                                              (p.bwd == BB_FAST_DEFERRED ? 0.0 : act_bytes(x) + grad_bytes(out) + grad_bytes(x));
    }
    return L3_OK;
}

void tower_forward(l3_engine* e, Tower& tw) {
    const bool training = tw.training;
    for (auto& op : tw.ops) {
        Tensor& x = tw.t[op.in];
        Tensor& y = tw.t[op.out];
        switch (op.kind) {
            case OP_CONV: {
                const ConvPlan& p = op.cp;
                ConvBufs b;
                b.x = x.d, b.w = e->params[op.p_kernel].d, b.bias = e->params[op.p_bias].d, b.y = y.d;
                b.wprep = op.wflip, b.wino_u = op.wino_uf;
                b.stat_part = p.stat_mode ? e->stat_scratch : nullptr, b.stat_mode = p.stat_mode;
                ProfScope ps(e, F_CONV_FWD, conv_flops(op.geom), op.name.c_str(), p.fwd.executed);
                ps.bytes(p.fwd_bytes);
                conv_run_fwd(p.fwd, op.geom, p.st, b, e->stream);
                break;
            }
            case OP_BN: {
                const BnPlan& p = op.bp;
                ProfScope ps(e, F_ELEMWISE, 0.0);
                ps.bytes(p.fwd_bytes);
                const float* gamma = e->params[op.p_gamma].d;
                const float* beta = e->params[op.p_beta].d;
                switch (p.stats) {
                    case BS_PARTIALS:
                        bn_stats_from_partials(e->stat_scratch, p.stat_blocks, e->params[op.bias_param].d, gamma, beta, op.mean, op.var,
                                               op.scale, op.shift, x.rows(), x.C, BN_EPS, op.prerelu ? 1 : 0, e->stream);
                        break;
                    case BS_FAST:
                        bn_stats_fast(x.d, gamma, beta, op.mean, op.var, op.scale, op.shift, e->red_scratch, x.rows(), x.C, BN_EPS,
                                      op.prerelu ? 1 : 0, e->stream, x.d_bf16 ? 1 : 0);
                        break;
                    case BS_PLAIN:
                        bn_stats(x.d, gamma, beta, op.mean, op.var, op.scale, op.shift, e->red_scratch, x.rows(), x.C, BN_EPS, e->stream);
                        break;
                    case BS_MOVING:
                        bn_scale_shift(gamma, beta, e->params[op.p_mmean].d, e->params[op.p_mvar].d, op.scale, op.shift, x.C, BN_EPS,
                                       e->stream);
                        break;
                }
                if (p.bwd == BB_BY_FIRST_CONV) bn_xhat_ones(x.d, op.mean, op.var, BN_EPS, (&op + 1)->xaug, x.rows(), x.C, e->stream);
                if (op.fuse_pool >= 0) {
                    Tensor& pl = tw.t[tw.ops[op.fuse_pool].out];
                    bn_relu_pool2_fwd(x.d, op.scale, op.shift, pl.d, x.N, x.H, x.W, x.C, pl.H, pl.W, pl.batch_stride,
                                      op.prerelu ? 2 : (op.fused_relu ? 1 : 0), e->stream, pl.d_bf16 ? 1 : 0, x.d_bf16 ? 1 : 0,
                                      training ? (void*)op.xwin : nullptr);
                } else if (y.d_bf16 || x.d_bf16) {
                    bn_apply_fast(x.d, op.scale, op.shift, y.d, x.rows(), x.C, op.fused_relu ? 1 : 0, e->stream, y.d_bf16 ? 1 : 0,
                                  x.d_bf16 ? 1 : 0);
                } else {
                    bn_apply(x.d, op.scale, op.shift, y.d, x.rows(), x.C, op.fused_relu ? 1 : 0, e->stream);
                }
                break;
            }
            case OP_RELU: {
                if (op.fused_into_bn) break;
                ProfScope ps(e, F_ELEMWISE, 0.0);
                ps.bytes(act_bytes(x) + act_bytes(y));
                relu_fwd(x.d, y.d, x.numel(), e->stream);
                break;
            }
            case OP_POOL: {
                if (op.fused_into_bn) break;
                ProfScope ps(e, F_ELEMWISE, 0.0);
                ps.bytes(act_bytes(x) + act_bytes(y));
                maxpool_fwd(x.d, y.d, op.pg, e->stream);
                break;
            }
            default: break;
        }
    }
}

BnBwdFuse bn_bwd_fuse(const Tower& tw, const Op& bn) {
    return BnBwdFuse{bn.fuse_pool >= 0 ? bn.xwin : tw.t[bn.in].d, bn.scale, bn.shift, bn.mean, bn.var, BN_EPS, bn.fused_relu ? 1 : 0};
}

void tower_backward_block(l3_engine* e, Tower& tw, int block) {
    const bool training = tw.training;
    for (int oi = (int)tw.ops.size() - 1; oi >= 0; --oi) {
        Op& op = tw.ops[oi];
        if (op.block != block) continue;
        Tensor& x = tw.t[op.in];
        Tensor& y = tw.t[op.out];
        switch (op.kind) {
            case OP_POOL: {
                if (op.fused_into_bn) break;
                ProfScope ps(e, F_ELEMWISE, 0.0);
                ps.bytes(act_bytes(x) + grad_bytes(y) + grad_bytes(x));
                maxpool_bwd(x.d, y.g, x.g, op.pg, e->stream);
                break;
            }
            case OP_RELU: {
                if (op.fused_into_bn) break;
                ProfScope ps(e, F_ELEMWISE, 0.0);
                ps.bytes(act_bytes(y) + grad_bytes(y) + grad_bytes(x));
                relu_bwd(y.d, y.g, x.g, x.numel(), e->stream);
                break;
            }
            case OP_BN: {
                const BnPlan& p = op.bp;
                if (p.bwd == BB_BY_FIRST_CONV) break;
                ProfScope ps(e, F_ELEMWISE, 0.0);
                ps.bytes(p.bwd_bytes);
                const float* mean = training ? op.mean : e->params[op.p_mmean].d;
                const float* var = training ? op.var : e->params[op.p_mvar].d;
                const float* gamma = e->params[op.p_gamma].d;
                float *dgamma = e->params[op.p_gamma].g, *dbeta = e->params[op.p_beta].g;
                if (p.bwd == BB_PLAIN) {
                    bn_bwd(x.d, y.d, y.g, gamma, mean, var, x.g, dgamma, dbeta, e->red_scratch, x.rows(), x.C, BN_EPS, op.fused_relu ? 1 : 0,
                           training ? 1 : 0, e->stream);
                    break;
                }
                const bool pooled = p.bwd == BB_FAST_POOLED, defer = p.bwd == BB_FAST_DEFERRED;
                const Tensor& dy = pooled ? tw.t[tw.ops[op.fuse_pool].out] : y;
                bn_bwd_fast(x.d, op.scale, op.shift, mean, var, gamma, dy.g, pooled ? 1 : 0, x.N, x.H, x.W, x.C, dy.H, dy.W,
                            pooled ? dy.batch_stride : (int64_t)x.H * x.W * x.C, defer ? nullptr : x.g, dgamma, dbeta,
                            defer ? nullptr : op.bias_param >= 0 ? e->params[op.bias_param].g : nullptr, e->red_scratch, BN_EPS,
                            pooled ? (op.prerelu ? 2 : 1) : (op.fused_relu ? 1 : 0), training ? 1 : 0, e->stream, x.g_bf16 ? 1 : 0,
                            x.d_bf16 ? 1 : 0, dy.g_bf16 ? 1 : 0, p.bwd_blocks > 0 ? e->stat_scratch : nullptr, p.bwd_blocks);
                break;
            }
            case OP_CONV: {
                const ConvPlan& p = op.cp;
                const float* w = e->params[op.p_kernel].d;
                if (p.aug != FW_NONE) {
                    ProfScope ps(e, F_CONV_WGRAD, conv_flops(op.geom), op.name.c_str());
                    ps.bytes(p.wg_bytes);
                    const Op& bn = tw.ops[op.in_bn];
                    if (p.aug == FW_AUG_DEFERRED) {
                        const Op& fb = tw.ops[op.bn_defer];
                        const Tensor &bi = tw.t[fb.in], &bo = tw.t[fb.out];
                        const float* co = bn_bwd_fast_coeffs(e->red_scratch, op.cout);
                        const FirstWgFuse f{bi.d, bo.g, fb.scale, fb.shift, co, co + op.cout, co + 2 * op.cout, fb.fused_relu ? 1 : 0,
                                            bi.d_bf16 ? 1 : 0};
                        conv_wgrad(op.xaug, nullptr, op.gaug, e->wg_scratch, op.ageom, e->stream, false, false, &f);
                    } else {
                        conv_wgrad(op.xaug, y.g, op.gaug, e->wg_scratch, op.ageom, e->stream);
                    }
                    first_conv_grads(op.gaug, w, e->params[bn.p_gamma].d, e->params[bn.p_beta].d, e->params[op.p_kernel].g,
                                     e->params[bn.p_gamma].g, e->params[bn.p_beta].g,
                                     op.bias_by_bn && p.aug == FW_AUG ? nullptr : e->params[op.p_bias].g, op.kh * op.kw, x.C, op.cout,
                                     e->stream);
                    break;
                }
                ConvBufs b;
                b.x = x.d, b.w = w, b.y = y.g, b.dx = x.g, b.dw = e->params[op.p_kernel].g;
                b.wprep = op.wflip, b.wino_u = op.wino_ud, b.wg_part = e->wg_scratch;
                {
                    ProfScope ps(e, F_CONV_WGRAD, conv_flops(op.geom), op.name.c_str(), p.wgrad.executed);
                    ps.bytes(p.wg_bytes);
                    conv_run_wgrad(p.wgrad, op.geom, b, e->stream);
                }
                if (p.colsum) {
                    ProfScope ps(e, F_ELEMWISE, 0.0);
                    ps.bytes(grad_bytes(y));
                    colsum(y.g, e->params[op.p_bias].g, e->red_scratch, y.rows(), y.C, e->stream);
                }
                if (p.dgrad.path == DG_NONE) break;
                ProfScope ps(e, F_CONV_DGRAD, conv_flops(op.geom), op.name.c_str(), p.dgrad.executed);
                ps.bytes(p.dg_bytes);
                BnBwdFuse bb{};
                if (p.bwd_bn >= 0) {
                    bb = bn_bwd_fuse(tw, tw.ops[p.bwd_bn]);
                    b.bn_bwd = &bb, b.stat_part = e->stat_scratch;
                }
                conv_run_dgrad(p.dgrad, op.geom, op.dgeom, p.st, b, e->stream);
                break;
            }
            default: break;
        }
    }
}

void l2_sums(l3_engine* e) {
    SumsqSegs segs{};
    int nl2 = 0;
    for (auto& s : e->segments) nl2 += s.l2 ? 1 : 0;
    if (nl2 <= SUMSQ_MAX_SEGS) {
        for (auto& s : e->segments)
            if (s.l2) {
                segs.off[segs.count] = s.off;
                segs.n[segs.count++] = s.n;
            }
        sumsq_multi(e->arena_p, segs, e->l2part, e->sq_scratch, e->stream);
        return;
    }
    int si = 0;
    for (auto& s : e->segments)
        if (s.l2) sumsq(e->arena_p + s.off, s.n, e->l2part + si++, e->sq_scratch, e->stream);
}

int forward_all(l3_engine* e, bool training) {
    int rc;
// ... 1383 lines not shown
    }
    int64_t D = 0;
    int rc = embed_check(e, false, pool_h, pool_w, &D);
    if (rc) return rc;
    if ((rc = embed_dest_check(e, fn, dst, n_frames, D))) return rc;
    int64_t bad = 0;
    if (const char* why = resample_clips_error(clips, n_clips, n_native, AUDIO_T, n_window, num_table, n_samples, true, &bad)) {
        e->err = name + ": " + (bad >= 0 ? "clip " + std::to_string(bad) + ": " : std::string()) + why;
        return L3_EINVAL;
    }
    if (const char* why = frame_table_error(table, n_frames, n_samples, &bad)) {
        e->err = name + ": frame " + std::to_string(bad) + ": " + why;
        return L3_EINVAL;
    }
    if (n_frames == 0) return L3_OK;
    HIPCHK(e, hipSetDevice(e->cfg.device));
    if ((rc = dev_grow_t(e, &e->clip_samples, &e->clip_samples_cap, (size_t)(n_samples > 0 ? n_samples : 1)))) return rc;
    if ((rc = dev_grow_t(e, &e->clip_table, &e->clip_table_cap, (size_t)n_frames * 3))) return rc;
    if ((rc = e->resample.run(native, n_native, clips, n_clips, AUDIO_T, half_window, n_window, num_table, true, e->clip_samples,
                              n_samples, e->stream, &e->err)))
        return rc;
    HIPCHK(e, hipMemcpyAsync(e->clip_table, table, (size_t)n_frames * 3 * 8, hipMemcpyHostToDevice, e->stream));
    EmbedSource src;
    src.samples = e->clip_samples;
    src.table = e->clip_table;
    return embed_rows(e, false, src, n_frames, pool_h, pool_w, D, dst);
}

int l3_embed_audio_clips_resampled(l3_engine* e, const float* native, int64_t n_native, const int64_t* clips, int64_t n_clips,
                                   const double* half_window, int64_t n_window, int num_table, int64_t n_samples,
                                   const int64_t* table, int64_t n_frames, int pool_h, int pool_w, float* out) {
    if (!e) return L3_EINVAL;
    EmbedDest dst;
    dst.host = out;
    return embed_clips_resampled_to(e, "l3_embed_audio_clips_resampled", native, n_native, clips, n_clips, half_window, n_window,
                                    num_table, n_samples, table, n_frames, pool_h, pool_w, dst);
}

int l3_embed_audio_clips_resampled_dev(l3_engine* e, const float* native, int64_t n_native, const int64_t* clips, int64_t n_clips,
                                       const double* half_window, int64_t n_window, int num_table, int64_t n_samples,
                                       const int64_t* table, int64_t n_frames, int pool_h, int pool_w, l3_feat* dst_feat,
                                       int64_t row0) {
    if (!e) return L3_EINVAL;
    EmbedDest dst;
    dst.dev = true, dst.feat = dst_feat, dst.row0 = row0;
    return embed_clips_resampled_to(e, "l3_embed_audio_clips_resampled_dev", native, n_native, clips, n_clips, half_window, n_window,
                                    num_table, n_samples, table, n_frames, pool_h, pool_w, dst);
}

int l3_activation_numel(l3_engine* e, const char* name, int64_t* numel) {
    if (!e || !name || !numel) return L3_EINVAL;
    const std::string nm(name);
    if (nm == "h0") { *numel = (int64_t)e->B * (e->nv + e->na); return L3_OK; }
    if (nm == "h1") { *numel = (int64_t)e->B * e->head; return L3_OK; }
    if (nm == "logits" || nm == "probs") { *numel = (int64_t)e->B * 2; return L3_OK; }
    Tensor* t = nullptr;
    if (!find_tower_tensor(e, nm, &t)) {
        e->err = "unknown activation: " + nm;
        return L3_EINVAL;
    }
    *numel = t->numel();
    return L3_OK;
}

int l3_get_activation(l3_engine* e, const char* name, float* dst, int64_t numel) {
    int64_t n = 0;
    int rc = l3_activation_numel(e, name, &n);
    if (rc) return rc;
    if (n != numel) {
        e->err = "activation size mismatch";
        return L3_EINVAL;
    }
    HIPCHK(e, hipSetDevice(e->cfg.device));
    HIPCHK(e, l3::stream_wait(e->stream));
    const std::string nm(name);
    const float* src = nullptr;
    if (nm == "h0") src = e->h0;
    else if (nm == "h1") src = e->h1;
    else if (nm == "logits") src = e->logits;
    else if (nm == "probs") src = e->probs;
    else {
        Tensor* t = nullptr;
        find_tower_tensor(e, nm, &t);
        if (t->alias || t->d == nullptr) {
            e->err = "activation is not materialised (aliased into h0 or fused away)";
            return L3_EINVAL;
        }
        src = t->d;
        if (t->d_bf16) {
            std::vector<uint16_t> h((size_t)numel);
            HIPCHK(e, hipMemcpy(h.data(), src, (size_t)numel * 2, hipMemcpyDeviceToHost));
            l3::widen_bf16(dst, h.data(), (size_t)numel);
            return L3_OK;
        }
    }
    HIPCHK(e, hipMemcpy(dst, src, (size_t)numel * 4, hipMemcpyDeviceToHost));
    return L3_OK;
}

int l3_sync(l3_engine* e) {
    if (!e) return L3_EINVAL;
    HIPCHK(e, hipSetDevice(e->cfg.device));
    HIPCHK(e, l3::stream_wait(e->stream));
    if (e->side) HIPCHK(e, l3::stream_wait(e->side));
    prof_collect(e);
    return L3_OK;
}

int l3_set_tower_overlap(l3_engine* e, int on) {
    if (!e) return L3_EINVAL;
    HIPCHK(e, l3::stream_wait(e->stream));
    if (e->side) HIPCHK(e, l3::stream_wait(e->side));
    e->overlap = on != 0;
    return L3_OK;
}

int l3_profile_enable(l3_engine* e, int on) {
    if (!e) return L3_EINVAL;
    HIPCHK(e, l3::stream_wait(e->stream));
    if (e->side) HIPCHK(e, l3::stream_wait(e->side));
    prof_collect(e);
    e->prof_on = on != 0;
    if (on)
        for (int i = 0; i < F_COUNT; ++i) {
            e->prof_ms[i] = 0;
            e->prof_n[i] = 0;
            e->prof_flops[i] = 0;
            e->prof_exec[i] = 0;
            e->prof_bytes[i] = 0;
        }
    return L3_OK;
}

int l3_profile_read(l3_engine* e, int family, double* ms, int64_t* launches, double* flops) {
    if (!e || family < 0 || family >= F_COUNT) return L3_EINVAL;
    HIPCHK(e, l3::stream_wait(e->stream));
    prof_collect(e);
    if (ms) *ms = e->prof_ms[family];
    if (launches) *launches = e->prof_n[family];
    if (flops) *flops = e->prof_flops[family];
    return L3_OK;
}

int l3_profile_read_bytes(l3_engine* e, int family, double* bytes) {
    if (!e || !bytes || family < 0 || family >= F_COUNT) return L3_EINVAL;
    HIPCHK(e, l3::stream_wait(e->stream));
    prof_collect(e);
    *bytes = e->prof_bytes[family];
    return L3_OK;
}

int l3_profile_read_executed(l3_engine* e, int family, double* flops) {
    if (!e || !flops || family < 0 || family >= F_COUNT) return L3_EINVAL;
    HIPCHK(e, l3::stream_wait(e->stream));
    prof_collect(e);
    *flops = e->prof_exec[family];
    return L3_OK;
}

}
```

### l3embedding_amd/csrc/kernels.h

```cpp
#pragma once
#include <hip/hip_runtime.h>
#include <stdint.h>

#include <string>
#include <vector>

#include "host_common.h"

namespace l3 {

struct ConvGeom {
    int N, H, W, Cin;
    int Ho, Wo, Cout;
    int KH, KW, padT, padL;
    int f2x2 = 0;
    int solo = 0;
    int dynamic = 0;
    float* tail_scratch = nullptr;
    size_t tail_scratch_bytes = 0;
};
size_t conv_wino4_tail_scratch_bytes();

struct BnBwdFuse {
    const float* x;
// ... 28 lines not shown
struct FirstWgFuse {
    const void *bnx, *dA;
    const float *scale, *shift;
    const float *cA, *cB, *cC;
    int relu;
    int bf16;
};
int conv_first_wgrad(const float* x, const float* dy, float* part, const ConvGeom& g, hipStream_t s, const FirstWgFuse* fuse = nullptr);
int conv_first_stat_blocks(const ConvGeom& g);
void conv_first_fwd(const float* x, const float* w, const float* bias, void* y, const ConvGeom& g, hipStream_t s,
                    float* stat_part = nullptr, int stat_mode = 0, bool out_bf16 = false);

bool conv_wgrad_wino_ok(const ConvGeom& g);
int conv_wgrad_wino_splits(const ConvGeom& g, int n);
int conv_wgrad_wino_max_splits(const ConvGeom& g, int n);
double conv_wgrad_wino_executed_flops(const ConvGeom& g);
void conv_wgrad_wino_launch(const float* x, const float* dy, float* part, const ConvGeom& g, int n, hipStream_t s);
void conv_wgrad_wino_finish(const float* part, float* dw, const ConvGeom& g, int splits, hipStream_t s);
double conv_wgrad_executed_flops(const ConvGeom& g, bool bf16);
bool conv_wgrad_bf16_tr_enabled();
void conv_wgrad_bf16_tr_launch(const void* x, const void* dy, float* part, const ConvGeom& g, int n, int splits, hipStream_t s);

bool conv_bf16_ok(const ConvGeom& g);
void conv_bf16_fwd(const float* x, const float* wn, const float* bias, float* y, const ConvGeom& g, hipStream_t s,
                   bool operands_bf16 = false, float* stat_part = nullptr, int stat_mode = 0, bool out_bf16 = false,
                   const BnBwdFuse* bn_bwd = nullptr);
int conv_bf16_stat_blocks(const ConvGeom& g);
bool conv_bf16_halo_ok(const ConvGeom& g);
int conv_bf16_halo_patches(const ConvGeom& g, int n);
void conv_bf16_halo_launch(const void* x, const void* wn, const float* bias, void* y, const ConvGeom& g, int n,
                           hipStream_t s, float* stat_part, int stat_mode, bool out_bf16, const BnBwdFuse* bn_bwd = nullptr);
void conv_weights_bf16(const float* w, void* out, int KH, int KW, int Cin, int Cout, bool flip, hipStream_t s);

void bn_xhat_ones(const float* x, const float* mean, const float* var, float eps, float* xa, int64_t rows, int C,
                  hipStream_t s);
void first_conv_grads(const float* gaug, const float* w, const float* gamma, const float* beta, float* dw, float* dgamma,
                      float* dbeta, float* dbias, int taps, int C, int Co, hipStream_t s);

size_t colreduce_scratch_floats(int64_t rows, int C);
void colsum(const float* x, float* out, float* scratch, int64_t rows, int C, hipStream_t s);
void bn_stats(const float* x, const float* gamma, const float* beta, float* mean, float* var,
              float* scale, float* shift, float* scratch, int64_t rows, int C, float eps,
              hipStream_t s);
void bn_scale_shift(const float* gamma, const float* beta, const float* mean, const float* var,
                    float* scale, float* shift, int C, float eps, hipStream_t s);
void bn_apply(const float* x, const float* scale, const float* shift, float* y, int64_t rows, int C,
              int relu, hipStream_t s);
void bn_bwd(const float* x, const float* y, const float* dy, const float* gamma, const float* mean,
            const float* var, float* dx, float* dgamma, float* dbeta, float* scratch, int64_t rows,
            int C, float eps, int relu, int training, hipStream_t s);
void bn_moving_update(float* moving, float* biased, const float* batch, int C, float momentum,
                      int zero_debias, int step, hipStream_t s);
int* persistent_work_counters(hipStream_t s);

struct BnMovingEntry {
    float* moving;
    float* biased;
    const float* batch;
    int C;
    int off;
};
void bn_moving_update_all(const BnMovingEntry* tab_dev, int entries, int max_c, float momentum, int zero_debias, int64_t step,
                          hipStream_t s, const float* gathered = nullptr, int replicas = 1, int64_t stride = 0);
void bn_moving_pack(const BnMovingEntry* tab_dev, int entries, int max_c, float* packed, hipStream_t s);

bool bn_fast_ok(int C);
size_t bn_fast_scratch_floats(int C);
void bn_stats_fast(const float* x, const float* gamma, const float* beta, float* mean, float* var, float* scale,
                   float* shift, float* scratch, int64_t rows, int C, float eps, int prerelu, hipStream_t s, int x_bf16 = 0);
void bn_stats_from_partials(const float* part, int nblk, const float* pivot, const float* gamma, const float* beta,
                            float* mean, float* var, float* scale, float* shift, int64_t rows, int C, float eps,
                            int prerelu, hipStream_t s);
void bn_apply_fast(const float* x, const float* scale, const float* shift, float* y, int64_t rows, int C, int relu,
                   hipStream_t s, int out_bf16 = 0, int x_bf16 = 0);
void bn_relu_pool2_fwd(const float* x, const float* scale, const float* shift, float* p, int N, int H, int W, int C,
                       int Ho, int Wo, int64_t out_batch_stride, int mode, hipStream_t s, int out_bf16 = 0, int x_bf16 = 0,
                       void* xwin = nullptr);
void bn_bwd_fast(const float* x, const float* scale, const float* shift, const float* mean, const float* var,
                 const float* gamma, const float* dy, int pooled, int N, int H, int W, int C, int Ho, int Wo,
                 int64_t dy_batch_stride, float* dx, float* dgamma, float* dbeta, float* dbias, float* scratch,
                 float eps, int relu, int training, hipStream_t s, int dx_bf16 = 0, int x_bf16 = 0, int dy_bf16 = 0,
                 const float* ready_part = nullptr, int ready_blocks = 0);
const float* bn_bwd_fast_coeffs(const float* scratch, int C);

void relu_fwd(const float* x, float* y, int64_t n, hipStream_t s);
void relu_bwd(const float* y, const float* dy, float* dx, int64_t n, hipStream_t s);

struct PoolGeom {
    int N, H, W, C, Ho, Wo, ph, pw, sh, sw, padT, padL;
    int64_t out_batch_stride;
};
void maxpool_fwd(const float* x, float* y, const PoolGeom& g, hipStream_t s);
void maxpool_bwd(const float* x, const float* dy, float* dx, const PoolGeom& g, hipStream_t s);

void preprocess_video(const uint8_t* u8, float* out, int64_t n, hipStream_t s);
void preprocess_audio(const int16_t* pcm, float* out, int64_t n, hipStream_t s);
void labels_onehot(const int32_t* lab, float* out, int64_t n, hipStream_t s);

struct AugmentParams {
    int32_t start_x, start_y, flip, sat_first;
    float saturation, brightness;
};
constexpr int AUG_CROP = 224;
void augment_video(const uint8_t* u8, int N, int H, int W, const AugmentParams* params, uint8_t* out_u8, float* out_f32,
                   hipStream_t s);
void augment_audio(const int16_t* pcm, int N, int T, const double* u, int16_t* out_i16, float* out_f32, double* gains,
                   hipStream_t s);

struct FrontendCfg {
    int n_dft, n_hop, pad_left, n_frames, n_freq, n_mels;
    int sqrt_out;
    int db;
    int loglambda;
    int ncols_pad;
    int folded, ke, ko, nc;
    int factored, N1, N2;
};
void dft_pack_frames(const float* audio, const float* win, float* a1, int B, int T, const FrontendCfg& c, hipStream_t s);
void dft_twiddle(const float* y, const float* tw, float* a2, float* nyq, int frames, const FrontendCfg& c, hipStream_t s);
void frame_audio_folded(const float* audio, float* fe, float* fo, int B, int T, const FrontendCfg& c, hipStream_t s);
void frame_audio(const float* audio, float* frames, int B, int T, const FrontendCfg& c, hipStream_t s);
void dft_fused(const float* audio, const float* win, const float* b1, const float* b2, const float* tw, const float* melw,
               const int* mel_start, const int* mel_len, const int* mel_off, float* out, int B, int T, const FrontendCfg& c,
               hipStream_t s);
void spec_to_features(const float* spec, const float* melw, const int* mel_start, const int* mel_len,
                      const int* mel_off, float* out, int B, const FrontendCfg& c, hipStream_t s, const float* nyq = nullptr);
void db_normalize(float* x, float* smax, int B, int64_t per_sample, int batch_scope, hipStream_t s);

void gather_frames(const float* samples, const int64_t* table, float* out, int rows, int n_real, int T, hipStream_t s);
inline const char* frame_table_error(const int64_t* table, int64_t n_frames, int64_t n_samples, int64_t* bad_row) {
    const int64_t lim = (int64_t)1 << 62;
    for (int64_t r = 0; r < n_frames; ++r) {
        const int64_t start = table[3 * r], lo = table[3 * r + 1], hi = table[3 * r + 2];
        *bad_row = r;
        if (lo < 0) return "lo < 0";
        if (lo > hi) return "lo > hi";
        if (hi > n_samples) return "hi > n_samples";
        if (start < -lim || start > lim) return "start out of range";
    }
    return nullptr;
}

constexpr int IMG = 224;
constexpr int IMAGE_ROW = 7;
constexpr int IMAGE_DESC = 4;
constexpr int64_t IMAGE_MAX_SIDE = 8192;
const char* image_table_error(const int64_t* table, int64_t n_frames, int64_t n_bytes, int64_t* bad_row);
struct ImagePlan {
    std::vector<int64_t> frames, taps;
};
void image_plan(const int64_t* table, int64_t n_frames, ImagePlan* plan);
void image_frames(const uint8_t* pixels, const int64_t* frames, const int64_t* taps, uint8_t* out_u8, float* out_f32, int rows,
                  int n_real, hipStream_t s);

constexpr int RESAMPLE_ROW = 6;
struct ResampleClip {
    int64_t x_off, L, sr_o, sr_n, t0, n_out, y_off;
    int64_t table;
};
struct ResamplePlan {
    std::vector<ResampleClip> clips;
    std::vector<int64_t> blocks;
};
struct ResampleTables {
    std::vector<double> window;
    std::vector<double> keys;
    std::vector<double> tables;
    uint64_t generation = 0;
};
int64_t resample_out_len(int64_t L, int64_t sr_o, int64_t sr_n);
const char* resample_clips_error(const int64_t* clips, int64_t n_clips, int64_t n_native, int64_t sr_new, int64_t n_window,
                                 int num_table, int64_t n_samples, bool copy_equal, int64_t* bad);
struct ResampleStage {
    int run(const float* native, int64_t n_native, const int64_t* clips, int64_t n_clips, int64_t sr_new,
// ... 76 lines not shown
```

### l3embedding_amd/csrc/ops.hip

```cpp
#include <hip/hip_runtime.h>

#include <cstring>
#include <string>
#include <vector>

#include "../../include/l3hip.h"
#include "conv_path.h"
#include "kernels.h"
#include "knobs.h"
#include "mlp.h"
#include "vggish.h"

namespace {
using namespace l3;

struct Scope {
    DeviceBufs bufs;
    hipStream_t s = nullptr;
    bool ok = true;
    explicit Scope(int device) : ok(device_ok(device)) {}
    ~Scope() { (void)hipDeviceSynchronize(); }
    template <class T>
    T* alloc(size_t count) {
        T* p = bufs.alloc<T>(count);
// ... 214 lines not shown
    } else {
        bn_bwd(d_x, d_y, d_dy, d_g, d_m, d_v, d_dx, d_dg, d_db, d_red, rows, c, 1e-3f, relu, 1, sc.s);
    }
    sc.get_stored(dx, d_dx, n, obf);
    sc.get(dgamma, d_dg, (size_t)c);
    sc.get(dbeta, d_db, (size_t)c);
    return sc.status();
}

static int pool2_common(int device, const float* x, const float* gamma, const float* beta, const float* dp, float* p,
                        float* mean, float* var, float* dx, float* dgamma, float* dbeta, float* dbias, int n, int h,
                        int wd, int c, int same, int mode, int x_bf16, float* xwin = nullptr) {
    if (!bn_fast_ok(c) || (mode != 1 && mode != 2)) return L3_EINVAL;
    Scope sc(device);
    if (!sc.ok) return L3_EHIP;
    const PoolGeom g = make_pool(n, h, wd, c, 2, 2, 2, 2, same);
    const size_t nx = (size_t)n * h * wd * c, np_ = (size_t)n * g.Ho * g.Wo * c;
    const bool obf = (x_bf16 & 4) != 0;
    float* d_x = sc.put(x, nx);
    float* d_g = sc.put(gamma, (size_t)c);
    float* d_b = sc.put(beta, (size_t)c);
    float *d_m = sc.alloc<float>(c), *d_v = sc.alloc<float>(c), *d_sc = sc.alloc<float>(c), *d_sh = sc.alloc<float>(c);
    float* d_p = sc.alloc<float>(np_);
    float* d_red = sc.alloc<float>(colreduce_scratch_floats((int64_t)n * h * wd, c));
    if (!sc.ok) return L3_ENOMEM;
    if (x_bf16 & 1) {
        uint16_t* xb = sc.alloc<uint16_t>(nx);
        if (!sc.ok) return L3_ENOMEM;
        cast_bf16(d_x, xb, (int64_t)nx, sc.s);
        d_x = reinterpret_cast<float*>(xb);
    }
    if (mode == 2 || (x_bf16 & 1))
        bn_stats_fast(d_x, d_g, d_b, d_m, d_v, d_sc, d_sh, d_red, (int64_t)n * h * wd, c, 1e-3f, mode == 2 ? 1 : 0, sc.s, x_bf16 & 1);
    else
        bn_stats(d_x, d_g, d_b, d_m, d_v, d_sc, d_sh, d_red, (int64_t)n * h * wd, c, 1e-3f, sc.s);
    float* d_win = xwin ? sc.alloc<float>(np_) : nullptr;
    if (!sc.ok) return L3_ENOMEM;
    bn_relu_pool2_fwd(d_x, d_sc, d_sh, d_p, n, h, wd, c, g.Ho, g.Wo, g.out_batch_stride, mode, sc.s, obf ? 1 : 0, x_bf16 & 1, d_win);
    sc.get_stored(p, d_p, np_, obf);
    if (xwin) sc.get_stored(xwin, d_win, np_, (x_bf16 & 1) != 0);
    sc.get(mean, d_m, (size_t)c);
    sc.get(var, d_v, (size_t)c);
    if (dp) {
        float* d_dp = sc.put(dp, np_);
        if (x_bf16 & 2) {
            uint16_t* gb = sc.alloc<uint16_t>(np_);
            if (!sc.ok) return L3_ENOMEM;
            cast_bf16(d_dp, gb, (int64_t)np_, sc.s);
            d_dp = reinterpret_cast<float*>(gb);
        }
        float* d_dx = sc.alloc<float>(nx);
        float *d_dg = sc.alloc<float>(c), *d_db = sc.alloc<float>(c), *d_dbias = sc.alloc<float>(c);
        if (!sc.ok) return L3_ENOMEM;
        bn_bwd_fast(d_x, d_sc, d_sh, d_m, d_v, d_g, d_dp, 1, n, h, wd, c, g.Ho, g.Wo, g.out_batch_stride, d_dx, d_dg,
                    d_db, d_dbias, d_red, 1e-3f, mode, 1, sc.s, obf ? 1 : 0, x_bf16 & 1, (x_bf16 & 2) ? 1 : 0);
        sc.get_stored(dx, d_dx, nx, obf);
        sc.get(dgamma, d_dg, (size_t)c);
        sc.get(dbeta, d_db, (size_t)c);
        sc.get(dbias, d_dbias, (size_t)c);
    }
    return sc.status();
}

int l3_op_bn_relu_pool2_fwd(int device, const float* x, const float* gamma, const float* beta, float* p, float* mean,
                            float* var, int n, int h, int wd, int c, int same, int relu_mode, int x_bf16) {
    return pool2_common(device, x, gamma, beta, nullptr, p, mean, var, nullptr, nullptr, nullptr, nullptr, n, h, wd, c,
                        same, relu_mode, x_bf16);
}

int l3_op_bn_relu_pool2_fwd_xwin(int device, const float* x, const float* gamma, const float* beta, float* p, float* mean,
                                 float* var, float* xwin, int n, int h, int wd, int c, int same, int relu_mode, int x_bf16) {
    if (!xwin) return L3_EINVAL;
    return pool2_common(device, x, gamma, beta, nullptr, p, mean, var, nullptr, nullptr, nullptr, nullptr, n, h, wd, c,
                        same, relu_mode, x_bf16, xwin);
}

int l3_op_bn_relu_pool2_bwd(int device, const float* x, const float* gamma, const float* beta, const float* dp,
                            float* dx, float* dgamma, float* dbeta, float* dbias, int n, int h, int wd, int c, int same,
                            int relu_mode, int x_bf16) {
    return pool2_common(device, x, gamma, beta, dp, nullptr, nullptr, nullptr, dx, dgamma, dbeta, dbias, n, h, wd, c,
                        same, relu_mode, x_bf16);
}

int l3_op_maxpool_fwd(int device, const float* x, float* y, int n, int h, int wd, int c, int ph, int pw, int sh,
                      int sw, int same) {
    Scope sc(device);
    if (!sc.ok) return L3_EHIP;
    const PoolGeom g = make_pool(n, h, wd, c, ph, pw, sh, sw, same);
    float* d_x = sc.put(x, (size_t)n * h * wd * c);
    float* d_y = sc.alloc<float>((size_t)n * g.Ho * g.Wo * c);
    if (!sc.ok) return L3_ENOMEM;
    maxpool_fwd(d_x, d_y, g, sc.s);
    sc.get(y, d_y, (size_t)n * g.Ho * g.Wo * c);
    return sc.status();
}

int l3_op_maxpool_bwd(int device, const float* x, const float* dy, float* dx, int n, int h, int wd, int c, int ph,
                      int pw, int sh, int sw, int same) {
    Scope sc(device);
    if (!sc.ok) return L3_EHIP;
    if (sh < ph || sw < pw) return L3_EINVAL;
    const PoolGeom g = make_pool(n, h, wd, c, ph, pw, sh, sw, same);
    float* d_x = sc.put(x, (size_t)n * h * wd * c);
    float* d_dy = sc.put(dy, (size_t)n * g.Ho * g.Wo * c);
    float* d_dx = sc.alloc<float>((size_t)n * h * wd * c);
    if (!sc.ok) return L3_ENOMEM;
    maxpool_bwd(d_x, d_dy, d_dx, g, sc.s);
    sc.get(dx, d_dx, (size_t)n * h * wd * c);
    return sc.status();
}

int l3_op_bn_stats_from_partials(int device, const float* part, int nblk, int c, const float* pivot, int64_t rows, float eps,
                                 float* mean, float* var) {
    Scope sc(device);
    if (!sc.ok) return L3_EHIP;
    if (nblk < 1 || c < 4 || c % 4) return L3_EINVAL;
    const size_t n = (size_t)nblk * 2 * c, guard = (size_t)8 * c;
    std::vector<float> host(n + guard);
    memcpy(host.data(), part, n * sizeof(float));
    for (size_t i = 0; i < guard; ++i) host[n + i] = -12345.f;
    float* d_part = sc.put(host.data(), n + guard);
    float* d_pivot = sc.put(pivot, (size_t)c);
    std::vector<float> ones((size_t)c, 1.f), zeros((size_t)c, 0.f);
    float* d_gamma = sc.put(ones.data(), (size_t)c);
    float* d_beta = sc.put(zeros.data(), (size_t)c);
    float* d_mean = sc.alloc<float>((size_t)c);
    float* d_var = sc.alloc<float>((size_t)c);
    float* d_scale = sc.alloc<float>((size_t)c);
    float* d_shift = sc.alloc<float>((size_t)c);
    if (!sc.ok) return L3_ENOMEM;
    bn_stats_from_partials(d_part, nblk, d_pivot, d_gamma, d_beta, d_mean, d_var, d_scale, d_shift, rows, c, eps, 0, sc.s);
    sc.get(mean, d_mean, (size_t)c);
    sc.get(var, d_var, (size_t)c);
    sc.get(host.data() + n, d_part + n, guard);
    for (size_t i = 0; i < guard; ++i)
        if (host[n + i] != -12345.f) return L3_EINVAL;
    return sc.status();
}

}

namespace {
struct GuardedPartials {
    static constexpr float SENTINEL = -12345.f;
    size_t n = 0, guard = 0, row = 0;
    float* dev = nullptr;
    std::vector<float> host;
    GuardedPartials(Scope& sc, int nblk, int c) {
        row = (size_t)2 * c;
        n = (size_t)nblk * 2 * c;
        guard = (size_t)(nblk > 8 ? nblk : 8) * 2 * c;
        host.assign(n + guard, SENTINEL);
        uint32_t nan_bits = 0x7fc00000u;
        float nan;
        memcpy(&nan, &nan_bits, sizeof nan);
        for (size_t i = 0; i < n; ++i) host[i] = nan;
        dev = sc.put(host.data(), n + guard);
    }
    int fetch(Scope& sc, const char* name, float* part) {
        sc.get(host.data(), dev, n + guard);
        if (!sc.ok) return L3_EHIP;
        if (const int rc = guard_check(name)) return rc;
        for (size_t i = 0; i < n; ++i)
            if (host[i] != host[i]) {
                set_op_error(std::string(name) + ": the epilogue left partial block " + std::to_string(i / row) + " unwritten");
                return L3_EINVAL;
// ... 852 lines not shown
```

Before: 2024 pairs/s.

## Fuse batchnorm+ReLU with the final global max-pool in forward and backward

Adds fused kernels that apply BN scale/shift, ReLU and global max-pool in one pass over the last conv activation. The forward pass records the winning value and position per sample and channel. The backward pass builds the BN gradient from those winners and scatters into dx, so the post-BN activation tensor is never materialised and the separate maxpool kernels are skipped. This removes a full-size activation write and read plus separate pool launches. In exchange it adds a two-stage scan/merge kernel, extra per-sample buffers, and a new planner path with tie-breaking semantics that may differ slightly from the original pool.

After: 2040 pairs/s, median of 6. Within noise of the previous version (+0.8%).

```diff
diff --git a/include/l3hip.h b/include/l3hip.h
--- a/include/l3hip.h
+++ b/include/l3hip.h
@@ -190,6 +190,10 @@
                               int relu, int64_t bn_rows);
 int l3_op_bn_relu_pool2_fwd_xwin(int device, const float *x, const float *gamma, const float *beta, float *p, float *mean,
                                  float *var, float *xwin, int n, int h, int wd, int c, int same, int relu_mode, int x_bf16);
+int l3_op_bn_relu_gpool_fwd(int device, const float *x, const float *gamma, const float *beta, float *h0, float *mean, float *var,
+                            float *xwin, int32_t *pos, int n, int h, int wd, int c, int64_t out_batch_stride);
+int l3_op_bn_relu_gpool_bwd(int device, const float *x, const float *gamma, const float *beta, const float *dh0, float *dx,
+                            float *dgamma, float *dbeta, float *dbias, int n, int h, int wd, int c, int64_t out_batch_stride);
 int l3_op_preprocess(int device, const uint8_t *video_u8, int64_t nv, float *video,
                      const int16_t *audio_i16, int64_t na, float *audio);
 int l3_op_augment_video(int device, const uint8_t *u8, int n, int h, int w, const l3_augment_params *params,
diff --git a/l3embedding_amd/_lib.py b/l3embedding_amd/_lib.py
--- a/l3embedding_amd/_lib.py
+++ b/l3embedding_amd/_lib.py
@@ -152,6 +152,8 @@
     'l3_op_conv2d_dgrad_bn_bwd': (C.c_int, [C.c_int, C.c_int] + [C.c_void_p] * 9 + [C.POINTER(C.c_int), C.c_void_p, C.c_void_p] +
                                   [C.c_int] * 9 + [C.c_int64]),
     'l3_op_bn_relu_pool2_fwd_xwin': (C.c_int, [C.c_int] + [C.c_void_p] * 7 + [C.c_int] * 7),
+    'l3_op_bn_relu_gpool_fwd': (C.c_int, [C.c_int] + [C.c_void_p] * 8 + [C.c_int] * 4 + [C.c_int64]),
+    'l3_op_bn_relu_gpool_bwd': (C.c_int, [C.c_int] + [C.c_void_p] * 8 + [C.c_int] * 4 + [C.c_int64]),
     'l3_op_preprocess': (C.c_int, [C.c_int, C.c_void_p, C.c_int64, C.c_void_p, C.c_void_p, C.c_int64, C.c_void_p]),
     'l3_op_augment_video': (C.c_int, [C.c_int, C.c_void_p, C.c_int, C.c_int, C.c_int, C.c_void_p, C.c_void_p, C.c_void_p]),
     'l3_op_augment_audio': (C.c_int, [C.c_int, C.c_void_p, C.c_int, C.c_int, C.c_void_p, C.c_void_p, C.c_void_p, C.c_void_p]),
@@ -835,6 +837,32 @@
     return dx, dg, db, dbias
 
 
+def op_bn_relu_gpool_fwd(x, gamma, beta, out_batch_stride=None, want_winners=True, fill=0.0, device=0):
+    lib = load()
+    x = _f32(x)
+    n, h, wd, c = x.shape
+    stride = c if out_batch_stride is None else int(out_batch_stride)
+    h0 = np.full((n, stride), fill, np.float32)
+    mean, var = np.empty((c,), np.float32), np.empty((c,), np.float32)
+    xwin = np.empty((n, c), np.float32) if want_winners else None
+    pos = np.empty((n, c), np.int32) if want_winners else None
+    check(lib.l3_op_bn_relu_gpool_fwd(device, _ptr(x), _ptr(_f32(gamma)), _ptr(_f32(beta)), _ptr(h0), _ptr(mean), _ptr(var),
+                                      _ptr(xwin), _ptr(pos), n, h, wd, c, stride))
+    return (h0, mean, var, xwin, pos) if want_winners else (h0, mean, var)
+
+
+def op_bn_relu_gpool_bwd(x, gamma, beta, dh0, device=0):
+    lib = load()
+    x, dh0 = _f32(x), _f32(dh0)
+    n, h, wd, c = x.shape
+    assert dh0.ndim == 2 and dh0.shape[0] == n
+    dx = np.empty_like(x)
+    dg, db, dbias = (np.empty((c,), np.float32) for _ in range(3))
+    check(lib.l3_op_bn_relu_gpool_bwd(device, _ptr(x), _ptr(_f32(gamma)), _ptr(_f32(beta)), _ptr(dh0), _ptr(dx), _ptr(dg), _ptr(db),
+                                      _ptr(dbias), n, h, wd, c, dh0.shape[1]))
+    return dx, dg, db, dbias
+
+
 def _pool_out(h, p, s, same):
     return -(-h // s) if same else (h - p) // s + 1
 
diff --git a/l3embedding_amd/csrc/bn_fused.hip b/l3embedding_amd/csrc/bn_fused.hip
--- a/l3embedding_amd/csrc/bn_fused.hip
+++ b/l3embedding_amd/csrc/bn_fused.hip
@@ -601,4 +601,216 @@
     if (dbias) launch_fast_final(SumFinal{dbias}, part, nb_a, C, s);
 }
 
-}
+constexpr int GP_U = 4;
+constexpr int GP_TILES = 8;
+constexpr int GP_NONE = 0x7fffffff;
+
+struct GPoolGeom {
+    int N, P, C4, lgC4;
+    int R;
+    int chunk, S;
+};
+
+bool bn_gpool_ok(int N, int H, int W, int C, int64_t out_batch_stride) {
+    return N >= 1 && H >= 1 && W >= 1 && bn_fast_ok(C) && C % 64 == 0 && FB % (C / 4) == 0 && out_batch_stride % 4 == 0 &&
+           out_batch_stride >= C && (int64_t)N * H * W < ((int64_t)1 << 31);
+}
+
+static GPoolGeom make_gpool(int N, int P, int C) {
+    GPoolGeom g;
+    g.N = N; g.P = P; g.C4 = C / 4;
+    g.lgC4 = 0;
+    while ((1 << g.lgC4) < g.C4) ++g.lgC4;
+    g.R = FB / g.C4;
+    g.chunk = g.R * GP_U * GP_TILES;
+    g.S = (P + g.chunk - 1) / g.chunk;
+    return g;
+}
+
+size_t bn_gpool_scratch_floats(int N, int H, int W, int C) {
+    const GPoolGeom g = make_gpool(N, H * W, C);
+    return (size_t)N * g.S * C * 2;
+}
+
+__global__ __launch_bounds__(FB) void bn_relu_gpool_scan_kernel(const float* __restrict__ x, const f32x4* scale, const f32x4* shift,
+                                                               float* __restrict__ pbest, int* __restrict__ parg, GPoolGeom g) {
+    __shared__ f32x4 sb[FB];
+    __shared__ i32x4 sa[FB];
+    const int t = threadIdx.x;
+    const int n = blockIdx.x / g.S, sl = blockIdx.x - n * g.S;
+    const int c4 = t & (g.C4 - 1), r = t >> g.lgC4;
+    const f32x4 sc = scale[c4], sh = shift[c4];
+    const int p0 = sl * g.chunk, p1 = p0 + g.chunk < g.P ? p0 + g.chunk : g.P;
+    const int64_t row0 = (int64_t)n * g.P;
+    f32x4 best = {-INFINITY, -INFINITY, -INFINITY, -INFINITY};
+    i32x4 arg = {GP_NONE, GP_NONE, GP_NONE, GP_NONE};
+    for (int pt = p0; pt < p1; pt += g.R * GP_U) {
+        f32x4 v[GP_U];
+#pragma unroll
+        for (int u = 0; u < GP_U; ++u) {
+            const int p = pt + u * g.R + r;
+            if (p < p1) v[u] = load_quad<false>(x, (row0 + p) * g.C4 + c4);
+        }
+#pragma unroll
+        for (int u = 0; u < GP_U; ++u) {
+            const int p = pt + u * g.R + r;
+            if (p >= p1) continue;
+            const f32x4 pre = bn_pre(v[u], sc, sh);
+#pragma unroll
+            for (int e = 0; e < 4; ++e)
+                if (pre[e] > best[e] || arg[e] == GP_NONE) {
+                    best[e] = pre[e];
+                    arg[e] = p;
+                }
+        }
+    }
+    sb[t] = best;
+    sa[t] = arg;
+    __syncthreads();
+    if (t < g.C4) {
+        for (int k = 1; k < g.R; ++k) {
+            const f32x4 vb = sb[k * g.C4 + t];
+            const i32x4 va = sa[k * g.C4 + t];
+#pragma unroll
+            for (int e = 0; e < 4; ++e)
+                if (vb[e] > best[e] || (vb[e] == best[e] && va[e] < arg[e]) || (arg[e] == GP_NONE && va[e] != GP_NONE)) {
+                    best[e] = vb[e];
+                    arg[e] = va[e];
+                }
+        }
+        const size_t o = (size_t)blockIdx.x * g.C4 + t;
+        reinterpret_cast<f32x4*>(pbest)[o] = best;
+        reinterpret_cast<i32x4*>(parg)[o] = arg;
+    }
+}
+
+__global__ __launch_bounds__(256) void bn_relu_gpool_merge_kernel(const float* __restrict__ x, const float* __restrict__ pbest,
+                                                                 const int* __restrict__ parg, float* __restrict__ h0,
+                                                                 int64_t out_batch_stride, float* __restrict__ xwin,
+                                                                 int* __restrict__ pos, GPoolGeom g) {
+    const int C = g.C4 * 4;
+    const int i = blockIdx.x * 256 + threadIdx.x;
+    if (i >= g.N * C) return;
+    const int n = i / C, c = i - n * C;
+    float b = -INFINITY;
+    int a = GP_NONE;
+    for (int sl = 0; sl < g.S; ++sl) {
+        const size_t o = ((size_t)n * g.S + sl) * C + c;
+        const float vb = pbest[o];
+        const int va = parg[o];
+        if (va != GP_NONE && (vb > b || a == GP_NONE)) {
+            b = vb;
+            a = va;
+        }
+    }
+    h0[(size_t)n * out_batch_stride + c] = fmaxf(b, 0.f);
+    if (a == GP_NONE) a = 0;
+    if (xwin != nullptr) {
+        xwin[i] = x[((size_t)n * g.P + a) * C + c];
+        pos[i] = a;
+    }
+}
+
+void bn_relu_gpool_fwd(const float* x, const float* scale, const float* shift, float* h0, int N, int H, int W, int C,
+                       int64_t out_batch_stride, float* xwin, int* pos, float* scratch, hipStream_t s) {
+    const GPoolGeom g = make_gpool(N, H * W, C);
+    float* pbest = scratch;
+    int* parg = reinterpret_cast<int*>(scratch + (size_t)N * g.S * C);
+    hipLaunchKernelGGL(bn_relu_gpool_scan_kernel, dim3(N * g.S), dim3(FB), 0, s, x, reinterpret_cast<const f32x4*>(scale),
+                       reinterpret_cast<const f32x4*>(shift), pbest, parg, g);
+    hipLaunchKernelGGL(bn_relu_gpool_merge_kernel, dim3((N * C + 255) / 256), dim3(256), 0, s, x, (const float*)pbest,
+                       (const int*)parg, h0, out_batch_stride, xwin, pos, g);
+}
+
+constexpr int GP_RED_SAMPLES = 8;
+__global__ __launch_bounds__(64) void bn_gpool_bwd_reduce_kernel(const float* __restrict__ xwin, const float* __restrict__ dy,
+                                                                int64_t dy_batch_stride, const float* scale, const float* shift,
+                                                                const float* mean, const float* var, float* __restrict__ part,
+                                                                int N, int C, int spb, float eps) {
+    const int c = blockIdx.x * 64 + threadIdx.x;
+    const float sc = scale[c], sh = shift[c], mu = mean[c], rs = rsqrtf(var[c] + eps);
+    const int n0 = blockIdx.y * spb, n1 = n0 + spb < N ? n0 + spb : N;
+    float a0 = 0.f, a1 = 0.f;
+    for (int n = n0; n < n1; ++n) {
+        const float xw = xwin[(size_t)n * C + c];
+        const float d = fmaf(xw, sc, sh) > 0.f ? dy[(size_t)n * dy_batch_stride + c] : 0.f;
+        a0 += d;
+        a1 += d * ((xw - mu) * rs);
+    }
+    part[((size_t)blockIdx.y * 2 + 0) * C + c] = a0;
+    part[((size_t)blockIdx.y * 2 + 1) * C + c] = a1;
+}
+
+void bn_gpool_bwd_reduce(const float* xwin, const float* scale, const float* shift, const float* mean, const float* var,
+                         const float* gamma, const float* dy, int64_t dy_batch_stride, int N, int H, int W, int C, float* dgamma,
+                         float* dbeta, float* scratch, float eps, int training, hipStream_t s) {
+    int spb = GP_RED_SAMPLES;
+    if ((N + spb - 1) / spb > FAST_MAX_BLOCKS) spb = (N + FAST_MAX_BLOCKS - 1) / FAST_MAX_BLOCKS;
+    const int nb = (N + spb - 1) / spb;
+    float* cA = scratch + (size_t)FAST_MAX_BLOCKS * 2 * C;
+    hipLaunchKernelGGL(bn_gpool_bwd_reduce_kernel, dim3(C / 64, nb), dim3(64), 0, s, xwin, dy, dy_batch_stride, scale, shift, mean,
+                       var, scratch, N, C, spb, eps);
+    launch_fast_final(BwdFinal{gamma, mean, var, dgamma, dbeta, cA, cA + C, cA + 2 * C, 1.0 / ((double)N * H * W), eps, training},
+                      scratch, nb, C, s);
+}
+
+__global__ __launch_bounds__(FB) void bn_gpool_bwd_apply_kernel(const float* __restrict__ x, const f32x4* __restrict__ xwin,
+                                                               const i32x4* __restrict__ pos, const float* __restrict__ dy,
+                                                               int64_t dy_bs4, const f32x4* scale, const f32x4* shift,
+                                                               const f32x4* cA, const f32x4* cB, const f32x4* cC,
+                                                               float* __restrict__ dx, float* part, int64_t n4, GPoolGeom g) {
+    const int c4 = (int)threadIdx.x & (g.C4 - 1);
+    const f32x4 sc = scale[c4], sh = shift[c4], A = cA[c4], B = cB[c4], Cc = cC[c4];
+    f32x4 a0 = {0.f, 0.f, 0.f, 0.f};
+    const int64_t stride = (int64_t)gridDim.x * (FB * GP_U);
+    for (int64_t q = (int64_t)blockIdx.x * (FB * GP_U) + threadIdx.x; q < n4; q += stride) {
+        f32x4 v[GP_U];
+        i32x4 w[GP_U];
+        int ns[GP_U], ps[GP_U];
+#pragma unroll
+        for (int u = 0; u < GP_U; ++u) {
+            const int64_t qu = q + u * FB;
+            if (qu >= n4) continue;
+            v[u] = load_quad<false>(x, qu);
+            const unsigned row = (unsigned)(qu >> g.lgC4);
+            const unsigned n = row / (unsigned)g.P;
+            ns[u] = (int)n;
+            ps[u] = (int)(row - n * (unsigned)g.P);
+            w[u] = pos[(size_t)n * g.C4 + c4];
+        }
+#pragma unroll
+        for (int u = 0; u < GP_U; ++u) {
+            const int64_t qu = q + u * FB;
+            if (qu >= n4) continue;
+            f32x4 d = {0.f, 0.f, 0.f, 0.f};
+            const int p = ps[u];
+            if (w[u].x == p || w[u].y == p || w[u].z == p || w[u].w == p) {
+                const f32x4 pre = bn_pre(xwin[(size_t)ns[u] * g.C4 + c4], sc, sh);
+                const f32x4 gr = *reinterpret_cast<const f32x4*>(dy + ((int64_t)ns[u] * dy_bs4 + c4) * 4);
+#pragma unroll
+                for (int e = 0; e < 4; ++e) d[e] = (w[u][e] == p && pre[e] > 0.f) ? gr[e] : 0.f;
+            }
+            const f32x4 o = A * d + (B * v[u] + Cc);
+            store_quad(dx, qu, o, 0);
+            a0 += o;
+        }
+    }
+    if (part != nullptr) block_write_partials(a0, a0, part, g.C4);
+}
+
+void bn_gpool_bwd_apply(const float* x, const float* xwin, const int* pos, const float* scale, const float* shift, const float* dy,
+                        int64_t dy_batch_stride, int N, int H, int W, int C, float* dx, float* dbias, float* scratch,
+                        hipStream_t s) {
+    const GPoolGeom g = make_gpool(N, H * W, C);
+    const int64_t n4 = (int64_t)N * H * W * g.C4;
+    int64_t nb = (n4 + FB * GP_U - 1) / (FB * GP_U);
+    if (nb > FAST_MAX_BLOCKS) nb = FAST_MAX_BLOCKS;
+    if (nb < 1) nb = 1;
+    const f32x4* cA = reinterpret_cast<const f32x4*>(scratch + (size_t)FAST_MAX_BLOCKS * 2 * C);
+    hipLaunchKernelGGL(bn_gpool_bwd_apply_kernel, dim3((int)nb), dim3(FB), 0, s, x, reinterpret_cast<const f32x4*>(xwin),
+                       reinterpret_cast<const i32x4*>(pos), dy, dy_batch_stride / 4, reinterpret_cast<const f32x4*>(scale),
+                       reinterpret_cast<const f32x4*>(shift), cA, cA + g.C4, cA + 2 * g.C4, dx, dbias ? scratch : nullptr, n4, g);
+    if (dbias) launch_fast_final(SumFinal{dbias}, scratch, (int)nb, C, s);
+}
+
+}
diff --git a/l3embedding_amd/csrc/elementwise.hip b/l3embedding_amd/csrc/elementwise.hip
--- a/l3embedding_amd/csrc/elementwise.hip
+++ b/l3embedding_amd/csrc/elementwise.hip
@@ -548,7 +548,7 @@
         *reinterpret_cast<gp4*>(dx + base + (size_t)p * C) = o;
     }
 }
-static bool is_global_pool(const PoolGeom& g) {
+bool is_global_pool(const PoolGeom& g) {
     return g.Ho == 1 && g.Wo == 1 && g.padT == 0 && g.padL == 0 && g.ph == g.H && g.pw == g.W && g.C % 64 == 0 &&
            g.out_batch_stride % 4 == 0;
 }
diff --git a/l3embedding_amd/csrc/engine.hip b/l3embedding_amd/csrc/engine.hip
--- a/l3embedding_amd/csrc/engine.hip
+++ b/l3embedding_amd/csrc/engine.hip
@@ -37,6 +37,7 @@
     int N = 0, H = 0, W = 0, C = 0;
     int64_t batch_stride = 0;
     bool alias = false;
+    bool skipped = false;
     bool d_bf16 = false, g_bf16 = false;
     int64_t numel() const { return (int64_t)N * H * W * C; }
     int64_t rows() const { return (int64_t)N * H * W; }
@@ -67,10 +68,11 @@
     double fwd_bytes = 0.0, wg_bytes = 0.0, dg_bytes = 0.0;
 };
 enum BnStats { BS_PARTIALS, BS_FAST, BS_PLAIN, BS_MOVING };
-enum BnBwd { BB_BY_FIRST_CONV, BB_FAST_POOLED, BB_FAST, BB_FAST_DEFERRED, BB_PLAIN };
+enum BnBwd { BB_BY_FIRST_CONV, BB_FAST_POOLED, BB_FAST_GPOOL, BB_FAST, BB_FAST_DEFERRED, BB_PLAIN };
 struct BnPlan {
     BnStats stats = BS_MOVING;
     int stat_blocks = 0;
+    bool gpool = false;
     BnBwd bwd = BB_PLAIN;
     int bwd_blocks = 0;
     double fwd_bytes = 0.0, bwd_bytes = 0.0;
@@ -102,6 +104,10 @@
     bool fused_relu = false;
     bool prerelu = false;
     int fuse_pool = -1;
+    int fuse_gpool = -1;
+    int gpool_bn = -1;
+    float* gp_xwin = nullptr;
+    int* gp_pos = nullptr;
     int bias_param = -1;
     bool fused_into_bn = false;
     bool bias_by_bn = false;
@@ -627,6 +633,14 @@
                 tw->ops[i - 2].bn_follow = (int)i;
                 op.fuse_pool = (int)i + 1;
                 tw->ops[i + 1].fused_into_bn = true;
+            }
+            if (op.fused_relu && !op.prerelu && op.fuse_pool < 0 && i + 1 < tw->ops.size() && tw->ops[i + 1].kind == OP_POOL &&
+                tw->ops[i + 1].in == op.out) {
+                const PoolGeom& pg = tw->ops[i + 1].pg;
+                if (is_global_pool(pg) && bn_gpool_ok(pg.N, pg.H, pg.W, pg.C, pg.out_batch_stride)) {
+                    op.fuse_gpool = (int)i + 1;
+                    tw->ops[i + 1].gpool_bn = (int)i;
+                }
             }
         }
     const int first_wg_fuse = knob_int("L3_FIRST_WG_FUSE", 1);
@@ -1041,6 +1055,12 @@
                 }
                 const size_t r = colreduce_scratch_floats(x.rows(), C);
                 if (r > red_max) red_max = r;
+                if (op.fuse_gpool >= 0 && !x.d_bf16 && !x.g_bf16) {
+                    if ((rc = dev_alloc_t(e, &op.gp_xwin, (size_t)x.N * C))) return rc;
+                    if ((rc = dev_alloc_t(e, &op.gp_pos, (size_t)x.N * C))) return rc;
+                    const size_t rg = bn_gpool_scratch_floats(x.N, x.H, x.W, C);
+                    if (rg > red_max) red_max = rg;
+                }
             }
         }
     }
@@ -1131,6 +1151,7 @@
 
 int plan_tower(l3_engine* e, Tower& tw, bool training, int solo) {
     static const int epi_stats = knob_int("L3_EPILOGUE_STATS", 1);
+    const int gpool_fuse = knob_int("L3_GPOOL_FUSE", 1);
     const bool bf16 = e->cfg.dtype == L3_DTYPE_BF16;
     tw.training = training;
     auto fits = [&](const Op& cv, int blocks, int C) {
@@ -1187,17 +1208,26 @@
     for (auto& op : tw.ops) {
         if (op.kind != OP_BN) continue;
         const Tensor &x = tw.t[op.in], &y = tw.t[op.out];
-        const Tensor& out = op.fuse_pool >= 0 ? tw.t[tw.ops[op.fuse_pool].out] : y;
         BnPlan& p = op.bp;
+        const Op* gp = op.fuse_gpool >= 0 ? &tw.ops[op.fuse_gpool] : nullptr;
+        p.gpool = gpool_fuse && gp != nullptr && op.gp_xwin != nullptr && !op.fused_first && is_global_pool(gp->pg) &&
+                  bn_gpool_ok(x.N, x.H, x.W, x.C, gp->pg.out_batch_stride);
+        tw.t[op.out].skipped = p.gpool;
+        const Tensor& out = op.fuse_pool >= 0 ? tw.t[tw.ops[op.fuse_pool].out] : p.gpool ? tw.t[gp->out] : y;
         p.stats = !training ? BS_MOVING : p.stat_blocks > 0 ? BS_PARTIALS : op.prerelu || x.d_bf16 ? BS_FAST : BS_PLAIN;
         p.bwd = training && op.fused_first ? BB_BY_FIRST_CONV : !bn_fast_ok(x.C) ? BB_PLAIN : op.fuse_pool >= 0 ? BB_FAST_POOLED
-                : defers(op) ? BB_FAST_DEFERRED : BB_FAST;
+                : p.gpool ? BB_FAST_GPOOL : defers(op) ? BB_FAST_DEFERRED : BB_FAST;
         p.fwd_bytes = (!training ? 0.0 : p.stat_blocks > 0 ? (double)p.stat_blocks * 2 * x.C * 4 : act_bytes(x)) + act_bytes(x) + act_bytes(out);
         if (p.bwd == BB_BY_FIRST_CONV) p.fwd_bytes += act_bytes(x) + (double)x.rows() * (&op + 1)->ageom.Cin * 4.0;
         if (op.fuse_pool >= 0 && training && op.xwin != nullptr) p.fwd_bytes += (double)out.numel() * (x.d_bf16 ? 2.0 : 4.0);
         p.bwd_bytes = p.bwd == BB_PLAIN ? 2.0 * (act_bytes(x) + grad_bytes(y)) + grad_bytes(x)
                                         : (p.bwd_blocks > 0 ? (double)p.bwd_blocks * 2 * x.C * 4 : act_bytes(x) + grad_bytes(out)) +
                                               (p.bwd == BB_FAST_DEFERRED ? 0.0 : act_bytes(x) + grad_bytes(out) + grad_bytes(x));
+        if (p.gpool) {
+            const double win = (double)out.numel() * 4.0;
+            p.fwd_bytes += 2.0 * win;
+            if (p.bwd == BB_FAST_GPOOL) p.bwd_bytes = win + grad_bytes(out) + act_bytes(x) + win + grad_bytes(x);
+        }
     }
     return L3_OK;
 }
@@ -1243,7 +1273,11 @@
                         break;
                 }
                 if (p.bwd == BB_BY_FIRST_CONV) bn_xhat_ones(x.d, op.mean, op.var, BN_EPS, (&op + 1)->xaug, x.rows(), x.C, e->stream);
-                if (op.fuse_pool >= 0) {
+                if (p.gpool) {
+                    const Tensor& pl = tw.t[tw.ops[op.fuse_gpool].out];
+                    bn_relu_gpool_fwd(x.d, op.scale, op.shift, pl.d, x.N, x.H, x.W, x.C, pl.batch_stride, op.gp_xwin, op.gp_pos,
+                                      e->red_scratch, e->stream);
+                } else if (op.fuse_pool >= 0) {
                     Tensor& pl = tw.t[tw.ops[op.fuse_pool].out];
                     bn_relu_pool2_fwd(x.d, op.scale, op.shift, pl.d, x.N, x.H, x.W, x.C, pl.H, pl.W, pl.batch_stride,
                                       op.prerelu ? 2 : (op.fused_relu ? 1 : 0), e->stream, pl.d_bf16 ? 1 : 0, x.d_bf16 ? 1 : 0,
@@ -1264,7 +1298,7 @@
                 break;
             }
             case OP_POOL: {
-                if (op.fused_into_bn) break;
+                if (op.fused_into_bn || (op.gpool_bn >= 0 && tw.ops[op.gpool_bn].bp.gpool)) break;
                 ProfScope ps(e, F_ELEMWISE, 0.0);
                 ps.bytes(act_bytes(x) + act_bytes(y));
                 maxpool_fwd(x.d, y.d, op.pg, e->stream);
@@ -1288,7 +1322,7 @@
         Tensor& y = tw.t[op.out];
         switch (op.kind) {
             case OP_POOL: {
-                if (op.fused_into_bn) break;
+                if (op.fused_into_bn || (op.gpool_bn >= 0 && tw.ops[op.gpool_bn].bp.gpool)) break;
                 ProfScope ps(e, F_ELEMWISE, 0.0);
                 ps.bytes(act_bytes(x) + grad_bytes(y) + grad_bytes(x));
                 maxpool_bwd(x.d, y.g, x.g, op.pg, e->stream);
@@ -1313,6 +1347,14 @@
                 if (p.bwd == BB_PLAIN) {
                     bn_bwd(x.d, y.d, y.g, gamma, mean, var, x.g, dgamma, dbeta, e->red_scratch, x.rows(), x.C, BN_EPS, op.fused_relu ? 1 : 0,
                            training ? 1 : 0, e->stream);
+                    break;
+                }
+                if (p.bwd == BB_FAST_GPOOL) {
+                    const Tensor& dy = tw.t[tw.ops[op.fuse_gpool].out];
+                    bn_gpool_bwd_reduce(op.gp_xwin, op.scale, op.shift, mean, var, gamma, dy.g, dy.batch_stride, x.N, x.H, x.W, x.C, dgamma,
+                                        dbeta, e->red_scratch, BN_EPS, training ? 1 : 0, e->stream);
+                    bn_gpool_bwd_apply(x.d, op.gp_xwin, op.gp_pos, op.scale, op.shift, dy.g, dy.batch_stride, x.N, x.H, x.W, x.C, x.g,
+                                       op.bias_param >= 0 ? e->params[op.bias_param].g : nullptr, e->red_scratch, e->stream);
                     break;
                 }
                 const bool pooled = p.bwd == BB_FAST_POOLED, defer = p.bwd == BB_FAST_DEFERRED;
@@ -2862,7 +2904,7 @@
     else {
         Tensor* t = nullptr;
         find_tower_tensor(e, nm, &t);
-        if (t->alias || t->d == nullptr) {
+        if (t->alias || t->d == nullptr || t->skipped) {
             e->err = "activation is not materialised (aliased into h0 or fused away)";
             return L3_EINVAL;
         }
diff --git a/l3embedding_amd/csrc/kernels.h b/l3embedding_amd/csrc/kernels.h
--- a/l3embedding_amd/csrc/kernels.h
+++ b/l3embedding_amd/csrc/kernels.h
@@ -134,6 +134,16 @@
                  float eps, int relu, int training, hipStream_t s, int dx_bf16 = 0, int x_bf16 = 0, int dy_bf16 = 0,
                  const float* ready_part = nullptr, int ready_blocks = 0);
 const float* bn_bwd_fast_coeffs(const float* scratch, int C);
+bool bn_gpool_ok(int N, int H, int W, int C, int64_t out_batch_stride);
+size_t bn_gpool_scratch_floats(int N, int H, int W, int C);
+void bn_relu_gpool_fwd(const float* x, const float* scale, const float* shift, float* h0, int N, int H, int W, int C,
+                       int64_t out_batch_stride, float* xwin, int* pos, float* scratch, hipStream_t s);
+void bn_gpool_bwd_reduce(const float* xwin, const float* scale, const float* shift, const float* mean, const float* var,
+                         const float* gamma, const float* dy, int64_t dy_batch_stride, int N, int H, int W, int C, float* dgamma,
+                         float* dbeta, float* scratch, float eps, int training, hipStream_t s);
+void bn_gpool_bwd_apply(const float* x, const float* xwin, const int* pos, const float* scale, const float* shift, const float* dy,
+                        int64_t dy_batch_stride, int N, int H, int W, int C, float* dx, float* dbias, float* scratch,
+                        hipStream_t s);
 
 void relu_fwd(const float* x, float* y, int64_t n, hipStream_t s);
 void relu_bwd(const float* y, const float* dy, float* dx, int64_t n, hipStream_t s);
@@ -142,6 +152,7 @@
     int N, H, W, C, Ho, Wo, ph, pw, sh, sw, padT, padL;
     int64_t out_batch_stride;
 };
+bool is_global_pool(const PoolGeom& g);
 void maxpool_fwd(const float* x, float* y, const PoolGeom& g, hipStream_t s);
 void maxpool_bwd(const float* x, const float* dy, float* dx, const PoolGeom& g, hipStream_t s);
 
diff --git a/l3embedding_amd/csrc/ops.hip b/l3embedding_amd/csrc/ops.hip
--- a/l3embedding_amd/csrc/ops.hip
+++ b/l3embedding_amd/csrc/ops.hip
@@ -320,6 +320,64 @@
                         same, relu_mode, x_bf16);
 }
 
+static int gpool_common(int device, const float* x, const float* gamma, const float* beta, const float* dh0, float* h0, float* mean,
+                        float* var, float* xwin, int32_t* pos, float* dx, float* dgamma, float* dbeta, float* dbias, int n, int h,
+                        int wd, int c, int64_t out_batch_stride) {
+    if (n < 1 || h < 1 || wd < 1 || !bn_gpool_ok(n, h, wd, c, out_batch_stride) || (xwin == nullptr) != (pos == nullptr))
+        return L3_EINVAL;
+    Scope sc(device);
+    if (!sc.ok) return L3_EHIP;
+    const size_t nx = (size_t)n * h * wd * c, nh = (size_t)n * out_batch_stride, nw = (size_t)n * c;
+    const bool win = xwin != nullptr || dh0 != nullptr;
+    float* d_x = sc.put(x, nx);
+    float* d_g = sc.put(gamma, (size_t)c);
+    float* d_b = sc.put(beta, (size_t)c);
+    float *d_m = sc.alloc<float>(c), *d_v = sc.alloc<float>(c), *d_sc = sc.alloc<float>(c), *d_sh = sc.alloc<float>(c);
+    float* d_h0 = h0 ? sc.put(h0, nh) : sc.alloc<float>(nh);
+    float* d_win = win ? sc.alloc<float>(nw) : nullptr;
+    int* d_pos = win ? sc.alloc<int>(nw) : nullptr;
+    size_t red = colreduce_scratch_floats((int64_t)n * h * wd, c);
+    if (bn_gpool_scratch_floats(n, h, wd, c) > red) red = bn_gpool_scratch_floats(n, h, wd, c);
+    float* d_red = sc.alloc<float>(red);
+    if (!sc.ok) return L3_ENOMEM;
+    bn_stats(d_x, d_g, d_b, d_m, d_v, d_sc, d_sh, d_red, (int64_t)n * h * wd, c, 1e-3f, sc.s);
+    bn_relu_gpool_fwd(d_x, d_sc, d_sh, d_h0, n, h, wd, c, out_batch_stride, d_win, d_pos, d_red, sc.s);
+    sc.get(h0, d_h0, nh);
+    sc.get(mean, d_m, (size_t)c);
+    sc.get(var, d_v, (size_t)c);
+    if (xwin) {
+        sc.get(xwin, d_win, nw);
+        sc.get(pos, d_pos, nw);
+    }
+    if (dh0) {
+        float* d_dh0 = sc.put(dh0, nh);
+        float* d_dx = sc.alloc<float>(nx);
+        float *d_dg = sc.alloc<float>(c), *d_db = sc.alloc<float>(c), *d_dbias = sc.alloc<float>(c);
+        if (!sc.ok) return L3_ENOMEM;
+        bn_gpool_bwd_reduce(d_win, d_sc, d_sh, d_m, d_v, d_g, d_dh0, out_batch_stride, n, h, wd, c, d_dg, d_db, d_red, 1e-3f, 1, sc.s);
+        bn_gpool_bwd_apply(d_x, d_win, d_pos, d_sc, d_sh, d_dh0, out_batch_stride, n, h, wd, c, d_dx, d_dbias, d_red, sc.s);
+        sc.get(dx, d_dx, nx);
+        sc.get(dgamma, d_dg, (size_t)c);
+        sc.get(dbeta, d_db, (size_t)c);
+        sc.get(dbias, d_dbias, (size_t)c);
+    }
+    return sc.status();
+}
+
+int l3_op_bn_relu_gpool_fwd(int device, const float* x, const float* gamma, const float* beta, float* h0, float* mean, float* var,
+                            float* xwin, int32_t* pos, int n, int h, int wd, int c, int64_t out_batch_stride) {
+    if (!h0) return L3_EINVAL;
+    return gpool_common(device, x, gamma, beta, nullptr, h0, mean, var, xwin, pos, nullptr, nullptr, nullptr, nullptr, n, h, wd, c,
+                        out_batch_stride);
+}
+
+int l3_op_bn_relu_gpool_bwd(int device, const float* x, const float* gamma, const float* beta, const float* dh0, float* dx,
+                            float* dgamma, float* dbeta, float* dbias, int n, int h, int wd, int c, int64_t out_batch_stride) {
+    if (!dh0) return L3_EINVAL;
+    return gpool_common(device, x, gamma, beta, dh0, nullptr, nullptr, nullptr, nullptr, nullptr, dx, dgamma, dbeta, dbias, n, h, wd,
+                        c, out_batch_stride);
+}
+
 int l3_op_maxpool_fwd(int device, const float* x, float* y, int n, int h, int wd, int c, int ph, int pw, int sh,
                       int sw, int same) {
     Scope sc(device);
```
